# liuhuang31/Megatts2_HierSpeechpp

Hardware: AMD Instinct MI355X
Metric: 16kHz audio samples/sec (whole node) + RTF, HierSpeech++ vocoder batch=32 (higher is better)
Workload: dtype f32; 1 GPU; vocoder-only infer(): 32 utterances x 4 s per GPU (BASELINE.json configs[1]), synthetic weights; batch_per_gpu=32, frames=200, global_batch=32, parallelism=dp1 (contiguous utterance shards of the global batch, one RCCL weight broadcast), launch_mode=hipGraph replay of the captured step

## Files before the change

include/hsp.h:

```cpp
#ifndef HSP_H_
#define HSP_H_

#include <stdint.h>

#ifdef __cplusplus
extern "C" {
#endif
#if defined(__GNUC__) || defined(__clang__)
#pragma GCC visibility push(default)
#endif

#define HSP_VERSION 104
#define HSP_EINVAL (-1)

int hsp_version(void);
const char* hsp_arch(void);


enum {
  HSP_PRO_NONE = 0,
  HSP_PRO_LRELU = 1,
  HSP_PRO_ACT1D = 2,
  HSP_PRO_SILU = 3
};

enum {
  HSP_ACT_NONE = 0,
  HSP_ACT_TANH = 1,
  HSP_ACT_GELU_TANH = 2,
  HSP_ACT_RELU = 3,
  HSP_ACT_MISH = 4,
  HSP_ACT_SILU = 5,
  HSP_ACT_SOFTPLUS = 6,
  HSP_ACT_GELU_ERF = 7
};

enum {
  HSP_ROWS_PLAIN = 0,
  HSP_ROWS_GATE_WN = 1,
  HSP_ROWS_GATE_GLU = 2,
  HSP_ROWS_SHUFFLE = 3
};

enum { HSP_MASK_NONE = 0, HSP_MASK_PRE = 1, HSP_MASK_POST = 2, HSP_MASK_BOTH = 3 };

typedef struct hsp_conv1d_args {
  const float* x;
  int64_t x_bs, x_cs, x_ts;
  int32_t B, Cin, Lin;
  const float* w;
  int32_t K, M, dil, pad, stride;
  const float* zeros;
  int32_t w_ld;
  float* y;
  int64_t y_bs, y_cs;
  int32_t Cout, Lout;
  int32_t ncols;
  int32_t prologue;
  float slope;
  const float* alpha_exp;
  const float* beta_inv;
  const float* filt;
  int32_t rows, gate_half, up, shuf_pad;
  const float* bias;
  const float* cbias;
  int64_t cbias_bs;
  int32_t act;
  const float* mask;
  int64_t mask_bs;
  int32_t mask_mode;
  const float* cscale;
  int64_t cscale_bs;
  float scale;
  const float* res;
  int64_t res_bs, res_cs;
  int32_t accumulate;
  float post_scale;
  int32_t debug;
  const float* ln_c1;
  float ln_eps;
  int32_t split_row;
  int32_t accumulate2;
  int32_t mask_mode2;
  float* y2;
  int64_t y2_bs, y2_cs;
  int64_t res_ts;
  int64_t w_bs;
  int32_t fold_cols;
} hsp_conv1d_args;

int hsp_conv1d_mfma_f32(const hsp_conv1d_args* a, void* stream);
int hsp_conv1d_direct_f32(const hsp_conv1d_args* a, void* stream);
int hsp_conv1d_mfma_plan(const hsp_conv1d_args* a, int32_t out4[4]);

int hsp_act_f32(const float* x, float* y, int64_t n, int32_t act, void* stream);
int hsp_reflect_pad_f32(const float* x, int64_t x_bs, float* y, int32_t B, int32_t L, int32_t pad, void* stream);
int hsp_f0_convert_f32(const float* f0_src, int32_t n_src, const float* f0_trg, int32_t n_trg, float* out, void* stream);

int hsp_reflect_pad_ragged_f32(const float* x, int64_t x_bs, const int64_t* lengths, float* y, int64_t y_bs, int32_t B,
                               int32_t L, int32_t pad, int32_t Lo, void* stream);
int hsp_f0_convert_batch_f32(const float* f0_src, int64_t src_bs, const int64_t* n_src, const float* f0_trg,
                             int64_t trg_bs, const int64_t* n_trg, int32_t nt_max, float* out, int64_t out_bs,
                             int32_t B, int32_t n_max, void* stream);
int hsp_stft_frames_ragged_f32(const float* x, int64_t x_bs, const int64_t* lengths, const float* window, float* frames,
                               int32_t B, int32_t L, int32_t n_fft, int32_t hop, int32_t T, int32_t f_ld, void* stream);
int hsp_abs_max_rows_f32(const float* x, int64_t x_bs, const int64_t* lengths, float* out, int32_t B, int64_t n,
                         void* stream);
int hsp_peak_int16_gains(const float* x, int64_t x_bs, const int64_t* lengths, const float* gains, int16_t* out,
                         int64_t o_bs, int32_t B, int64_t n, void* stream);

int hsp_mag_pha_f32(const float* spec, int64_t s_ld, float* mag, float* pha, int32_t n_freqs, int32_t T, float compress,
                    void* stream);
int hsp_lsigmoid_mul_f32(const float* m, const float* slope, float beta, const float* mag, float* out, int32_t T,
                         int32_t F, void* stream);
int hsp_atan2_f32(const float* y, const float* x, float* out, int64_t n, void* stream);
int hsp_polar_f32(const float* mag, const float* pha, float power, float* re, int64_t re_ld, float* im, int64_t im_ld,
                  int32_t F, int32_t T, void* stream);

int hsp_norm_factor_rows_f32(const float* x, int64_t x_bs, const int64_t* lengths, float* scale, float* inv, int32_t B,
                             int64_t L, void* stream);
int hsp_stft_frames_packed_f32(const float* x, int64_t x_bs, const int64_t* lengths, const float* scale,
                               const float* window, float* frames, const int32_t* seg, const int32_t* seg_host, int32_t B,
                               int64_t L, int32_t n_fft, int32_t hop, int32_t T_tot, int32_t f_ld, void* stream);
int hsp_instnorm_prelu_seg_f32(float* x, int64_t x_cs, int32_t C, int32_t T_tot, int32_t F, const int32_t* seg,
                               const int32_t* seg_host, int32_t B, const float* gamma, const float* beta,
                               const float* slope, float eps, void* stream);
int hsp_zero_gaps_f32(float* x, int64_t x_cs, int32_t C, int32_t T_tot, int32_t F, const int32_t* seg,
                      const int32_t* seg_host, int32_t B, void* stream);
int hsp_dwconv_bn_silu_seg_f32(const float* x, const float* w, const float* bias, const float* bn_weight,
                               const float* bn_bias, const float* bn_mean, const float* bn_var, float bn_eps, float* y,
                               int32_t A, int32_t C, int32_t N, int32_t K, const int32_t* seg, const int32_t* seg_host,
                               int32_t B, void* stream);
int hsp_istft_ola_seg_f32(const float* frames, int64_t f_ld, const float* window, const float* inv, float* out,
                          int64_t out_bs, int64_t n_max, int32_t n_fft, int32_t hop, const int32_t* seg,
                          const int32_t* seg_host, int32_t B, int32_t T_tot, void* stream);

int hsp_act1d_snakebeta_f32(const float* x, float* y, int32_t B, int32_t C, int32_t L,
                            const float* alpha_exp, const float* beta_inv, const float* filt,
                            void* stream);
int hsp_act1d_snakebeta_ragged_f32(const float* x, float* y, int32_t B, int32_t C, int32_t L, const int64_t* lens,
                                   const float* alpha_exp, const float* beta_inv, const float* filt, void* stream);
int hsp_snake_consts_f32(const float* alpha_log, const float* beta_log, float* alpha_exp,
                         float* beta_inv, int32_t C, void* stream);

int hsp_fold_weight_norm_f32(const float* v, const float* g, float* w, int32_t rows, int32_t cols,
                             void* stream);
int hsp_gather_f32(const float* src, const int32_t* map, float* dst, int64_t n, void* stream);

int hsp_sequence_mask_f32(const int64_t* length, float* mask, int32_t B, int32_t T, void* stream);
int hsp_flip_channels_f32(const float* x, float* y, int32_t B, int32_t C, int32_t T, void* stream);
int hsp_sample_prior_f32(const float* stats, const float* noise, const float* mask, float* z,
                         int32_t B, int32_t C, int32_t T, float noise_scale, void* stream);
int hsp_layernorm_mod_f32(const float* x, float* y, int32_t B, int32_t C, int32_t T, float eps,
                          const float* mask, const float* shift, const float* scale, int64_t mod_bs,
                          const float* gamma, const float* beta, void* stream);
typedef struct hsp_mha_args {
  const float *q, *k, *v;
  float* o;
  int64_t q_bs, k_bs, v_bs, o_bs;
  int32_t B, H, D, Tq, Tk;
  float qk_scale;
  const float* mask_q;
  const float* mask_k;
  const float* rel_k;
  const float* rel_v;
  int32_t window;
  int64_t q_cs, k_cs, v_cs, o_cs;
  const float* mask_dense;
  int64_t mask_dense_bs;
} hsp_mha_args;
int hsp_mha_f32(const hsp_mha_args* a, void* stream);
#define HSP_MHA_TOK 0
#define HSP_MHA_MFMA_WHOLE 1
#define HSP_MHA_MFMA_SLAB 2
#define HSP_MHA_MFMA_STREAM 3
#define HSP_MHA_ROW 4
#define HSP_MHA_ROW_STREAM 5
int hsp_mha_plan(const hsp_mha_args* a, int32_t out4[4]);
typedef struct hsp_mha_proj_args {
  const float *q, *k, *v;
  int64_t q_bs, q_cs, k_bs, k_cs, v_bs, v_cs;
  int32_t B, H, D, Tq, Tk;
  float qk_scale;
  const float* wt;
  int32_t M, wt_ld;
  const float* bias;
  const float* mask;
// ... 232 lines not shown
```

megatts2_hierspeechpp_amd/_lib.py:

```python
from __future__ import annotations

import ctypes as C
import os
from typing import Optional

import torch

_HERE = os.path.dirname(os.path.abspath(__file__))
LIB_PATH = os.environ.get("HSP_LIB", os.path.join(_HERE, "libhsp.so"))

PRO_NONE, PRO_LRELU, PRO_ACT1D, PRO_SILU = 0, 1, 2, 3
ACT_NONE, ACT_TANH, ACT_GELU_TANH, ACT_RELU, ACT_MISH, ACT_SILU, ACT_SOFTPLUS, ACT_GELU_ERF = 0, 1, 2, 3, 4, 5, 6, 7
ROWS_PLAIN, ROWS_GATE_WN, ROWS_GATE_GLU, ROWS_SHUFFLE = 0, 1, 2, 3
MASK_NONE, MASK_PRE, MASK_POST, MASK_BOTH = 0, 1, 2, 3
EINVAL = -1
MHA_TOK, MHA_MFMA_WHOLE, MHA_MFMA_SLAB, MHA_MFMA_STREAM, MHA_ROW, MHA_ROW_STREAM = range(6)

_fp = C.c_void_p


class Conv1dArgs(C.Structure):
    _fields_ = [
        ("x", _fp), ("x_bs", C.c_int64), ("x_cs", C.c_int64), ("x_ts", C.c_int64),
        ("B", C.c_int32), ("Cin", C.c_int32), ("Lin", C.c_int32),
        ("w", _fp), ("K", C.c_int32), ("M", C.c_int32), ("dil", C.c_int32), ("pad", C.c_int32), ("stride", C.c_int32),
        ("zeros", _fp), ("w_ld", C.c_int32),
        ("y", _fp), ("y_bs", C.c_int64), ("y_cs", C.c_int64),
        ("Cout", C.c_int32), ("Lout", C.c_int32), ("ncols", C.c_int32),
        ("prologue", C.c_int32), ("slope", C.c_float),
        ("alpha_exp", _fp), ("beta_inv", _fp), ("filt", _fp),
        ("rows", C.c_int32), ("gate_half", C.c_int32), ("up", C.c_int32), ("shuf_pad", C.c_int32),
        ("bias", _fp), ("cbias", _fp), ("cbias_bs", C.c_int64),
        ("act", C.c_int32),
        ("mask", _fp), ("mask_bs", C.c_int64), ("mask_mode", C.c_int32),
        ("cscale", _fp), ("cscale_bs", C.c_int64), ("scale", C.c_float),
        ("res", _fp), ("res_bs", C.c_int64), ("res_cs", C.c_int64),
        ("accumulate", C.c_int32), ("post_scale", C.c_float), ("debug", C.c_int32),
        ("ln_c1", _fp), ("ln_eps", C.c_float),
        ("split_row", C.c_int32), ("accumulate2", C.c_int32), ("mask_mode2", C.c_int32), ("y2", _fp),
        ("y2_bs", C.c_int64), ("y2_cs", C.c_int64), ("res_ts", C.c_int64), ("w_bs", C.c_int64),
        ("fold_cols", C.c_int32),
    ]


class MhaArgs(C.Structure):
    _fields_ = [
        ("q", _fp), ("k", _fp), ("v", _fp), ("o", _fp),
        ("q_bs", C.c_int64), ("k_bs", C.c_int64), ("v_bs", C.c_int64), ("o_bs", C.c_int64),
        ("B", C.c_int32), ("H", C.c_int32), ("D", C.c_int32), ("Tq", C.c_int32), ("Tk", C.c_int32),
        ("qk_scale", C.c_float),
        ("mask_q", _fp), ("mask_k", _fp), ("rel_k", _fp), ("rel_v", _fp), ("window", C.c_int32),
        ("q_cs", C.c_int64), ("k_cs", C.c_int64), ("v_cs", C.c_int64), ("o_cs", C.c_int64),
        ("mask_dense", _fp), ("mask_dense_bs", C.c_int64),
    ]


class MhaProjArgs(C.Structure):
    _fields_ = [
        ("q", _fp), ("k", _fp), ("v", _fp),
        ("q_bs", C.c_int64), ("q_cs", C.c_int64), ("k_bs", C.c_int64), ("k_cs", C.c_int64), ("v_bs", C.c_int64),
        ("v_cs", C.c_int64),
        ("B", C.c_int32), ("H", C.c_int32), ("D", C.c_int32), ("Tq", C.c_int32), ("Tk", C.c_int32),
        ("qk_scale", C.c_float),
        ("wt", _fp), ("M", C.c_int32), ("wt_ld", C.c_int32),
        ("bias", _fp), ("mask", _fp), ("mask_bs", C.c_int64), ("cscale", _fp), ("cscale_bs", C.c_int64),
        ("res", _fp), ("res_bs", C.c_int64), ("res_cs", C.c_int64), ("res_ts", C.c_int64),
        ("y", _fp), ("y_bs", C.c_int64), ("y_cs", C.c_int64), ("y_ts", C.c_int64), ("debug", C.c_int32),
        ("key_len", _fp),
    ]


class DftSegArgs(C.Structure):
    _fields_ = [
        ("x", _fp), ("x_bs", C.c_int64), ("x_cs", C.c_int64),
        ("y", _fp), ("y_bs", C.c_int64), ("y_cs", C.c_int64),
        ("B", C.c_int32), ("C", C.c_int32), ("L", C.c_int32),
        ("k", C.c_int32), ("dil", C.c_int32), ("pad", C.c_int32), ("nseg", C.c_int32), ("Np", C.c_int32),
        ("xf", _fp), ("xf_bs", C.c_int64), ("dft", _fp),
        ("bias", _fp), ("res", _fp), ("res_bs", C.c_int64), ("res_cs", C.c_int64),
        ("accumulate", C.c_int32), ("post_scale", C.c_float),
        ("act_alpha_exp", _fp), ("act_beta_inv", _fp), ("act_filt", _fp), ("prod3", C.c_int32),
        ("act_len", _fp),
    ]


class Cprod3Args(C.Structure):
    _fields_ = [
        ("xf", _fp), ("yf", _fp), ("w", _fp), ("zeros", _fp), ("xf_bs", C.c_int64), ("yf_bs", C.c_int64),
        ("bins", C.c_int32), ("C", C.c_int32), ("Np", C.c_int32), ("debug", C.c_int32),
    ]


class SampleArgs(C.Structure):
    _fields_ = [
        ("temperature", C.c_float), ("top_k", C.c_int32), ("top_p", C.c_float), ("repetition_penalty", C.c_float),
        ("seeds", _fp), ("probs", _fp), ("probs_bs", C.c_int64),
    ]


class PlmDecodeArgs(C.Structure):
    _fields_ = [
        ("x", _fp), ("x_bs", C.c_int64), ("x_cs", C.c_int64),
        ("y", _fp), ("y_bs", C.c_int64), ("y_cs", C.c_int64),
        ("k_cache", _fp), ("v_cache", _fp), ("bs", C.c_int64), ("cs", C.c_int64),
        ("t", C.c_int32), ("B", C.c_int32), ("D", C.c_int32), ("H", C.c_int32), ("F", C.c_int32), ("eps", C.c_float),
        ("g1", _fp), ("b1", _fp), ("wqkv_t", _fp), ("bqkv", _fp), ("wo_t", _fp), ("bo", _fp), ("g2", _fp), ("b2", _fp),
        ("w1_t", _fp), ("c1", _fp), ("w2_t", _fp), ("c2", _fp),
        ("workspace", _fp), ("workspace_bytes", C.c_int64), ("debug", C.c_int32),
    ]


class PlmPrefillAttnArgs(C.Structure):
    _fields_ = [
        ("qkv", _fp), ("q_rs", C.c_int64), ("out", _fp), ("o_rs", C.c_int64),
        ("k_cache", _fp), ("v_cache", _fp), ("cs", C.c_int64),
        ("n", C.c_int32), ("D", C.c_int32), ("H", C.c_int32), ("debug", C.c_int32),
    ]


class ProsodyArgs(C.Structure):
    _fields_ = [
        ("x", _fp), ("x_bs", C.c_int64), ("x_cs", C.c_int64), ("lengths", _fp),
        ("B", C.c_int32), ("D", C.c_int32), ("T", C.c_int32), ("k", C.c_int32), ("w_ld", C.c_int32), ("bins", C.c_int32),
        ("w1a", _fp), ("b1a", _fp), ("w1b", _fp), ("b1b", _fp), ("w2a", _fp), ("b2a", _fp), ("w2b", _fp), ("b2b", _fp),
        ("embed", _fp), ("codes", _fp), ("c_bs", C.c_int64), ("pooled", _fp), ("p_bs", C.c_int64),
    ]


class LimiterArgs(C.Structure):
    _fields_ = [
        ("x", _fp), ("x_bs", C.c_int64), ("lengths", _fp), ("gains", _fp), ("B", C.c_int32), ("n", C.c_int64),
        ("bank", _fp), ("F", C.c_int32), ("Z", C.c_int32), ("W", C.c_int32), ("ceiling", C.c_float),
        ("y", _fp), ("y_bs", C.c_int64), ("min_gain", _fp), ("tp", _fp),
    ]


WSPEC_BLOCK, WSPEC_THREE = 0, 1


SIGNATURES = {
    "hsp_version": (C.c_int, []),
    "hsp_arch": (C.c_char_p, []),
    "hsp_conv1d_mfma_f32": (C.c_int, [C.POINTER(Conv1dArgs), _fp]),
    "hsp_conv1d_direct_f32": (C.c_int, [C.POINTER(Conv1dArgs), _fp]),
    "hsp_conv1d_mfma_plan": (C.c_int, [C.POINTER(Conv1dArgs), C.POINTER(C.c_int32 * 4)]),
    "hsp_act1d_snakebeta_f32": (C.c_int, [_fp, _fp, C.c_int32, C.c_int32, C.c_int32, _fp, _fp, _fp, _fp]),
    "hsp_act1d_snakebeta_ragged_f32": (C.c_int, [_fp, _fp, C.c_int32, C.c_int32, C.c_int32, _fp, _fp, _fp, _fp, _fp]),
    "hsp_snake_consts_f32": (C.c_int, [_fp, _fp, _fp, _fp, C.c_int32, _fp]),
    "hsp_fold_weight_norm_f32": (C.c_int, [_fp, _fp, _fp, C.c_int32, C.c_int32, _fp]),
    "hsp_gather_f32": (C.c_int, [_fp, _fp, _fp, C.c_int64, _fp]),
    "hsp_sequence_mask_f32": (C.c_int, [_fp, _fp, C.c_int32, C.c_int32, _fp]),
    "hsp_flip_channels_f32": (C.c_int, [_fp, _fp, C.c_int32, C.c_int32, C.c_int32, _fp]),
    "hsp_sample_prior_f32": (C.c_int, [_fp, _fp, _fp, _fp, C.c_int32, C.c_int32, C.c_int32, C.c_float, _fp]),
    "hsp_layernorm_mod_f32": (C.c_int, [_fp, _fp, C.c_int32, C.c_int32, C.c_int32, C.c_float, _fp, _fp, _fp,
                                        C.c_int64, _fp, _fp, _fp]),
    "hsp_mha_f32": (C.c_int, [C.POINTER(MhaArgs), _fp]),
    "hsp_mha_plan": (C.c_int, [C.POINTER(MhaArgs), C.POINTER(C.c_int32 * 4)]),
    "hsp_mha_proj_f32": (C.c_int, [C.POINTER(MhaProjArgs), _fp]),
    "hsp_dftseg_fwd_f32": (C.c_int, [C.POINTER(DftSegArgs), _fp]),
    "hsp_dftseg_inv_f32": (C.c_int, [C.POINTER(DftSegArgs), _fp]),
    "hsp_dftseg_tables_f32": (C.c_int, [_fp, _fp]),
    "hsp_dftseg_pair_supported": (C.c_int, [C.POINTER(DftSegArgs), C.POINTER(DftSegArgs)]),
    "hsp_dftseg_pair_f32": (C.c_int, [C.POINTER(DftSegArgs), C.POINTER(DftSegArgs), _fp]),
    "hsp_dftseg_supported": (C.c_int, [C.POINTER(DftSegArgs)]),
    "hsp_cprod3_f32": (C.c_int, [C.POINTER(Cprod3Args), _fp]),
# ... 158 lines not shown
```

megatts2_hierspeechpp_amd/csrc/hsp_conv1d_consume.h:

```cpp
#pragma once

namespace hspconv {

__device__ __forceinline__ unsigned lds_addr(const float* p) {
  return (unsigned)(size_t)(const __attribute__((address_space(3))) float*)p;
}

template <int N, int I = 0>
__device__ __forceinline__ void ds_read_frags(float (&f)[N], unsigned addr) {
  if constexpr (I < N) {
    asm volatile("ds_read_b32 %0, %1 offset:%2" : "=v"(f[I]) : "v"(addr), "n"(I * 128));
    ds_read_frags<N, I + 1>(f, addr);
  }
}

template <int N, int OFF, int I = 0>
__device__ __forceinline__ void ds_read_frags_at(float (&f)[N], unsigned addr) {
  if constexpr (I < N) {
    static_assert(OFF + I * 128 < 65536, "ds_read immediate offsets are 16 bits");
    asm volatile("ds_read_b32 %0, %1 offset:%2" : "=v"(f[I]) : "v"(addr), "n"(OFF + I * 128));
    ds_read_frags_at<N, OFF, I + 1>(f, addr);
  }
}

template <int N, int I = 0>
__device__ __forceinline__ void bind_frags(float (&f)[N]) {
  if constexpr (I < N) {
    asm volatile("" : "+v"(f[I]));
    bind_frags<N, I + 1>(f);
  }
}
template <int NA, int NB>
__device__ __forceinline__ void wait_frags(float (&fa)[NA], float (&fb)[NB]) {
  asm volatile("s_waitcnt lgkmcnt(0)" ::: "memory");
  bind_frags<NA>(fa);
  bind_frags<NB>(fb);
}

template <class C, int EPI, bool ACT, int TM, int TN, bool FOLD = false>
__device__ __forceinline__ void conv_consume(const hsp_conv1d_args& a, const LdsPlan& P, float* const lds, const int b,
                                             const int m0, const int t0, const int p0, const int wm, const int wn,
                                             const int lane, const int nchunks, const int lkc, const int xvec,
                                             const int ks = 0, const int ts0 = 0) {
  static_assert(!FOLD || (TN == 1 && C::kKS == 1 && EPI != HSP_EPI_SHUF && !ACT), "folded columns: one column per lane, plain kernels");
  __builtin_assume(nchunks > 0);
  ConsLane L;
  L.lane = lane, L.l32 = lane & 31, L.half = lane >> 5;
  L.slot = wm * C::kWN + wn;
  L.mw = m0 + wm * (TM * 32), L.wcol = wn * (TN * 32);
  L.b = b, L.t0 = t0, L.ts0 = ts0;
  L.bl = b, L.tw = t0 + L.wcol + L.l32;
  int piece;
  fold_lane<FOLD>(a, b, ts0, L.wcol + L.l32, L.bl, L.tw, piece);
  L.xfold = 8 * piece + 4 - a.pad;

  f32x16 acc[TM][TN];
  {
  const int mw = L.mw, half = L.half, tw = L.tw, bl = L.bl;
  static_assert(C::kKS == 1 || EPI != HSP_EPI_INIT, "a K split with the accumulator-init epilogue would add the residual once per group");
  if constexpr (EPI == HSP_EPI_INIT) {
    const int rcs = (int)a.res_cs, ycs = (int)a.y_cs;
    const int lrow = mw + 4 * half;
    int tcl[TN];
#pragma unroll
    for (int n = 0; n < TN; ++n) tcl[n] = min(tw + n * 32, a.ncols - 1);
    auto init = [&](auto full_tag) __attribute__((always_inline)) {
      constexpr bool FULL = decltype(full_tag)::value;
      auto vec1 = [&](const float* p, int c) __attribute__((always_inline)) -> float {
        if constexpr (FULL) return (p + c)[lrow];
        else return p[min(lrow + c, a.Cout - 1)];
      };
      auto mat = [&](const float* p, int c, int cs, int n) __attribute__((always_inline)) -> float {
        if constexpr (FULL) return (p + c * cs)[lrow * cs + tcl[n]];
        else return p[min(lrow + c, a.Cout - 1) * cs + tcl[n]];
      };
      float add[TM][16];
      if (a.bias) {
        static_for<TM>([&](auto ii) __attribute__((always_inline)) {
          constexpr int i = decltype(ii)::value;
          static_for<16>([&](auto rr) __attribute__((always_inline)) {
            constexpr int r = decltype(rr)::value;
            add[i][r] = vec1(a.bias, i * 32 + HSP_ACC_ROW(r, 0));
          });
        });
      } else {
#pragma unroll
        for (int i = 0; i < TM; ++i)
#pragma unroll
          for (int r = 0; r < 16; ++r) add[i][r] = 0.0f;
      }
      if (a.res) {
        const float* const rb = a.res + (int64_t)bl * a.res_bs;
        static_for<TM>([&](auto ii) __attribute__((always_inline)) {
          constexpr int i = decltype(ii)::value;
          static_for<16>([&](auto rr) __attribute__((always_inline)) {
            constexpr int r = decltype(rr)::value;
            static_for<TN>([&](auto nn) __attribute__((always_inline)) {
              constexpr int n = decltype(nn)::value;
              acc[i][n][r] = mat(rb, i * 32 + HSP_ACC_ROW(r, 0), rcs, n);
            });
          });
        });
      } else {
#pragma unroll
        for (int i = 0; i < TM; ++i)
#pragma unroll
          for (int n = 0; n < TN; ++n)
#pragma unroll
            for (int r = 0; r < 16; ++r) acc[i][n][r] = 0.0f;
      }
      static_for<TM>([&](auto ii) __attribute__((always_inline)) {
        constexpr int i = decltype(ii)::value;
        static_for<TN>([&](auto nn) __attribute__((always_inline)) {
          constexpr int n = decltype(nn)::value;
          static_for<16>([&](auto rr) __attribute__((always_inline)) {
            constexpr int r = decltype(rr)::value;
            acc[i][n][r] += add[i][r];
          });
        });
      });
      if (a.cbias) {
        const float* const cb = a.cbias + (int64_t)bl * a.cbias_bs;
        static_for<TM>([&](auto ii) __attribute__((always_inline)) {
          constexpr int i = decltype(ii)::value;
          static_for<16>([&](auto rr) __attribute__((always_inline)) {
            constexpr int r = decltype(rr)::value;
            const float c = vec1(cb, i * 32 + HSP_ACC_ROW(r, 0));
            static_for<TN>([&](auto nn) __attribute__((always_inline)) {
              constexpr int n = decltype(nn)::value;
              acc[i][n][r] += c;
            });
          });
        });
      }
      if (a.accumulate) {
        const float* const yb = a.y + (int64_t)bl * a.y_bs;
        static_for<TM>([&](auto ii) __attribute__((always_inline)) {
          constexpr int i = decltype(ii)::value;
          static_for<TN>([&](auto nn) __attribute__((always_inline)) {
            constexpr int n = decltype(nn)::value;
            float tmp[16];
            static_for<16>([&](auto rr) __attribute__((always_inline)) {
              constexpr int r = decltype(rr)::value;
              tmp[r] = mat(yb, i * 32 + HSP_ACC_ROW(r, 0), ycs, n);
            });
            __builtin_amdgcn_sched_barrier(0);
            static_for<16>([&](auto rr) __attribute__((always_inline)) {
              constexpr int r = decltype(rr)::value;
              acc[i][n][r] += tmp[r];
            });
            __builtin_amdgcn_sched_barrier(0);
          });
        });
      }
    };
    if (mw + TM * 32 <= a.Cout) {
      init(std::true_type{});
    } else if (mw < a.Cout) {
      init(std::false_type{});
    } else {
#pragma unroll
      for (int i = 0; i < TM; ++i)
#pragma unroll
        for (int n = 0; n < TN; ++n)
#pragma unroll
          for (int r = 0; r < 16; ++r) acc[i][n][r] = 0.0f;
    }
  } else {
#pragma unroll
    for (int i = 0; i < TM; ++i)
#pragma unroll
      for (int j = 0; j < TN; ++j)
#pragma unroll
        for (int r = 0; r < 16; ++r) acc[i][j][r] = 0.0f;
  }
  }
  const int wlane = L.half * C::BM + wm * (TM * 32) + L.l32;
  const int xlane = L.half * P.xwp + L.wcol + L.l32 + (FOLD ? L.xfold : (xvec ? (p0 & 3) : 0));

  {
    constexpr int BM = C::BM;
    const int KC = P.kc;
    const int nsteps = ((a.K * KC) >> 1) / C::kKS;

    HSP_BARRIER(a);
    constexpr int kStepA = 2 * BM * 4;
    constexpr int rowB = 2 * C::XWP * 4;
    const int spanB = (KC >> 1) * rowB;
    const int tapB = 4 * a.dil;
    float fa0[TM], fb0[TN], fa1[TM], fb1[TN];
    auto mma_set = [&](const float (&fa)[TM], const float (&fb)[TN]) __attribute__((always_inline)) {
#pragma unroll
      for (int i = 0; i < TM; ++i)
#pragma unroll
        for (int n = 0; n < TN; ++n)
          acc[i][n] = __builtin_amdgcn_mfma_f32_32x32x2f32(fa[i], fb[n], acc[i][n], 0, 0, 0);
    };
    unsigned aA = lds_addr(lds + wlane);
    unsigned aB = lds_addr(lds + P.xa_off + xlane);
    int offA0 = 0, pairB0 = 0, tapoff0 = 0;
    if constexpr (C::kKS > 1) {
      const int s0 = ks * nsteps;
      offA0 = s0 * kStepA;
      pairB0 = (s0 & ((KC >> 1) - 1)) * rowB;
      tapoff0 = (s0 >> (lkc - 1)) * tapB;
    }
    unsigned va = aA + (unsigned)offA0, vb = aB + (unsigned)(pairB0 + tapoff0);
    const bool run = !HSP_DBG(a, HSP_CV_NO_MFMA);
    if (run) {
      ds_read_frags<TM>(fa0, va);
      ds_read_frags<TN>(fb0, vb);
    }
    for (int c = 0; c < nchunks; ++c) {
      if (!run) {
        HSP_BARRIER(a);
        continue;
      }
      int offA = offA0, pairB = pairB0, tapoff = tapoff0;
      int offB = 0;
      auto advance = [&]() __attribute__((always_inline)) {
        int t;
        asm volatile(
            "s_add_i32 %[oa], %[oa], %[sa]\n\t"
            "s_add_i32 %[pb], %[pb], %[sb]\n\t"
            "s_cmp_eq_u32 %[pb], %[span]\n\t"
            "s_cselect_b32 %[pb], 0, %[pb]\n\t"
            "s_cselect_b32 %[t], %[tap], 0\n\t"
            "s_add_i32 %[to], %[to], %[t]"
            : [oa] "+s"(offA), [pb] "+s"(pairB), [to] "+s"(tapoff), [t] "=&s"(t)
            : [sa] "n"(2 * kStepA), [sb] "n"(2 * rowB), [span] "s"(spanB), [tap] "s"(tapB)
            : "scc");
        offB = pairB + tapoff;
      };
      auto slot_a = [&](bool walk) __attribute__((always_inline)) {
        wait_frags(fa0, fb0);
        __builtin_amdgcn_sched_barrier(0);
        if (walk) advance();
        ds_read_frags_at<TM, kStepA>(fa1, va);
        ds_read_frags_at<TN, rowB>(fb1, vb);
        __builtin_amdgcn_sched_barrier(0);
        mma_set(fa0, fb0);
        __builtin_amdgcn_sched_barrier(0);
      };
      for (int s = 0; s + 2 < nsteps; s += 2) {
        slot_a(true);
        wait_frags(fa1, fb1);
        __builtin_amdgcn_sched_barrier(0);
        va = aA + (unsigned)offA;
        vb = aB + (unsigned)offB;
        ds_read_frags<TM>(fa0, va);
        ds_read_frags<TN>(fb0, vb);
        __builtin_amdgcn_sched_barrier(0);
        mma_set(fa1, fb1);
        __builtin_amdgcn_sched_barrier(0);
      }
      slot_a(false);
      HSP_BARRIER(a);
      bind_frags<TM>(fa1);
      bind_frags<TN>(fb1);
      if (c + 1 < nchunks) {
        const int nb = (c + 1) & 1;
        aA = lds_addr(lds + nb * P.ws_sz + wlane);
        aB = lds_addr(lds + P.xa_off + nb * P.xa_sz + xlane);
        va = aA + (unsigned)offA0;
        vb = aB + (unsigned)(pairB0 + tapoff0);
        __builtin_amdgcn_sched_barrier(0);
        ds_read_frags<TM>(fa0, va);
        ds_read_frags<TN>(fb0, vb);
      }
      __builtin_amdgcn_sched_barrier(0);
      mma_set(fa1, fb1);
      __builtin_amdgcn_sched_barrier(0);
    }
  }

  if constexpr (C::kKS > 1) {
    static_assert(C::kKS == 2, "one partner group per wave");
    float* const red = lds + C::kWM * C::kWN * (32 * 36) + (wm * C::kWN + wn) * (TM * TN * 16 * 64) + lane;
    if (ks > 0) {
      for_acc<TM, TN>([&](auto ii, auto nn, auto rr) __attribute__((always_inline)) {
        constexpr int i = ii, n = nn, r = rr;
        red[((i * TN + n) * 16 + r) * 64] = acc[i][n][r];
      });
    }
    lds_barrier();
    if (ks > 0) return;
    for_acc<TM, TN>([&](auto ii, auto nn, auto rr) __attribute__((always_inline)) {
      constexpr int i = ii, n = nn, r = rr;
      acc[i][n][r] += red[((i * TN + n) * 16 + r) * 64];
    });
  }
  if (HSP_DBG(a, HSP_CV_NO_EPILOGUE)) return;
  if constexpr (EPI == HSP_EPI_INIT) {
    const int mw = L.mw, half = L.half, tw = L.tw, bl = L.bl;
    float* const yb = a.y + (int64_t)bl * a.y_bs;
    const int ycs = (int)a.y_cs;
    const bool full = mw + TM * 32 <= a.Cout &&
                      t0 + wn * (TN * 32) + TN * 32 <= (FOLD ? a.B * a.ncols : a.ncols);
    const float ps = a.post_scale;
    if (full) {
      const int lrow = mw + 4 * half;
      int voff[TN];
#pragma unroll
      for (int n = 0; n < TN; ++n) voff[n] = lrow * ycs + tw + n * 32;
      static_for<TM>([&](auto ii) __attribute__((always_inline)) {
        constexpr int i = decltype(ii)::value;
        static_for<16>([&](auto rr) __attribute__((always_inline)) {
          constexpr int r = decltype(rr)::value;
          float* const yp = yb + (i * 32 + HSP_ACC_ROW(r, 0)) * ycs;
          static_for<TN>([&](auto nn) __attribute__((always_inline)) {
            constexpr int n = decltype(nn)::value;
            if (HSP_DBG(a, HSP_CV_NT_STORES)) __builtin_nontemporal_store(acc[i][n][r] * ps, yp + voff[n]);
            else yp[voff[n]] = acc[i][n][r] * ps;
          });
        });
      });
    } else {
      static_for<TM>([&](auto ii) __attribute__((always_inline)) {
        constexpr int i = decltype(ii)::value;
        static_for<TN>([&](auto nn) __attribute__((always_inline)) {
          constexpr int n = decltype(nn)::value;
          const int t = tw + n * 32;
          static_for<16>([&](auto rr) __attribute__((always_inline)) {
            constexpr int r = decltype(rr)::value;
            const int row = mw + i * 32 + HSP_ACC_ROW(r, half);
            if (row < a.Cout && t < a.ncols) yb[row * ycs + t] = acc[i][n][r] * ps;
          });
        });
      });
    }
  }
  else if constexpr (EPI == HSP_EPI_VEC) epi_vec<FOLD>(a, L, lds, acc);
  else if constexpr (EPI == HSP_EPI_GATE) epi_gate(a, L, acc);
  else if constexpr (EPI == HSP_EPI_SHUF) epi_shuf(a, L, acc);
  else epi_gen(a, L, acc);
}

}
```

megatts2_hierspeechpp_amd/csrc/hsp_conv1d_direct.hip:

```cpp
#include <type_traits>
#include "hsp_device.h"

namespace {

__global__ __launch_bounds__(256) void conv1d_direct_kernel(const hsp_conv1d_args a) {
  const int64_t total = (int64_t)a.B * a.Cout * a.Lout;
  for (int64_t idx = (int64_t)blockIdx.x * blockDim.x + threadIdx.x; idx < total;
       idx += (int64_t)gridDim.x * blockDim.x) {
    const int t = (int)(idx % a.Lout);
    const int64_t r = idx / a.Lout;
    const int co = (int)(r % a.Cout);
    const int b = (int)(r / a.Cout);
    const float* xb = a.x + (int64_t)b * a.x_bs;
    float acc = 0.0f;
    for (int j = 0; j < a.K; ++j) {
      const int p = t * a.stride + j * a.dil - a.pad;
      if (p < 0 || p >= a.Lin) continue;
      const float* wj = a.w + (int64_t)j * a.Cin * a.w_ld + co;
      const float* xp = xb + (int64_t)p * a.x_ts;
      if (a.prologue == HSP_PRO_NONE) {
        float acc4[4] = {0.f, 0.f, 0.f, 0.f};
        int ci = 0;
        for (; ci + 8 <= a.Cin; ci += 8) {
          float wv[8], xv[8];
// ... 33 lines not shown
    f(std::integral_constant<int, N - 1>{});
  }
}

template <int K>
__global__ __launch_bounds__(256) void conv1d_cout1_kernel(const hsp_conv1d_args a, int n_tiles) {
  constexpr int H = (K - 1) / 2, CU = 4;
  __shared__ float ws[C1_MAXW];
  for (int e = threadIdx.x; e < a.Cin * K; e += 256) {
    const int c = e / K, j = e - c * K;
    ws[e] = a.w[((int64_t)j * a.Cin + c) * a.w_ld];
  }
  __syncthreads();
  const int tile = blockIdx.x % n_tiles, b = blockIdx.x / n_tiles;
  const int t = tile * 1024 + 4 * threadIdx.x;
  if (t >= a.Lout) return;
  const int L = a.Lin;
  const float* xb = a.x + (int64_t)b * a.x_bs + t;
  const int64_t xcs = a.x_cs;
  float acc0 = 0.f, acc1 = 0.f, acc2 = 0.f, acc3 = 0.f;
  const bool lo = t - 4 >= 0, hi = t + 4 < L;
  const int offl = lo ? -4 : 0, offh = hi ? 4 : 0;
  const int ngroups = a.Cin / CU;
  for (int g = 0; g < ngroups; ++g) {
    const float* xc = xb + (int64_t)(g * CU) * xcs;
    float4 va[CU], vb[CU], vc[CU];
    c1_static_for<CU>([&](auto uu) __attribute__((always_inline)) {
      constexpr int u = decltype(uu)::value;
      va[u] = *reinterpret_cast<const float4*>(xc + u * xcs + offl);
      vb[u] = *reinterpret_cast<const float4*>(xc + u * xcs);
      vc[u] = *reinterpret_cast<const float4*>(xc + u * xcs + offh);
    });
    c1_static_for<CU>([&](auto uu) __attribute__((always_inline)) {
      constexpr int u = decltype(uu)::value;
      const float w_[12] = {lo ? va[u].x : 0.f, lo ? va[u].y : 0.f, lo ? va[u].z : 0.f, lo ? va[u].w : 0.f,
                            vb[u].x, vb[u].y, vb[u].z, vb[u].w,
                            hi ? vc[u].x : 0.f, hi ? vc[u].y : 0.f, hi ? vc[u].z : 0.f, hi ? vc[u].w : 0.f};
      const float* wc = ws + (g * CU + u) * K;
      c1_static_for<K>([&](auto jj) __attribute__((always_inline)) {
        constexpr int j = decltype(jj)::value;
        const float wj = wc[j];
        acc0 = fmaf(wj, w_[4 + j - H], acc0);
        acc1 = fmaf(wj, w_[5 + j - H], acc1);
        acc2 = fmaf(wj, w_[6 + j - H], acc2);
        acc3 = fmaf(wj, w_[7 + j - H], acc3);
      });
    });
  }
  for (int c = ngroups * CU; c < a.Cin; ++c) {
    const float* xc = xb + (int64_t)c * xcs;
    const float4 va = *reinterpret_cast<const float4*>(xc + offl);
    const float4 vb = *reinterpret_cast<const float4*>(xc);
    const float4 vc = *reinterpret_cast<const float4*>(xc + offh);
    const float w_[12] = {lo ? va.x : 0.f, lo ? va.y : 0.f, lo ? va.z : 0.f, lo ? va.w : 0.f, vb.x, vb.y, vb.z, vb.w,
                          hi ? vc.x : 0.f, hi ? vc.y : 0.f, hi ? vc.z : 0.f, hi ? vc.w : 0.f};
    const float* wc = ws + c * K;
    c1_static_for<K>([&](auto jj) __attribute__((always_inline)) {
      constexpr int j = decltype(jj)::value;
      const float wj = wc[j];
      acc0 = fmaf(wj, w_[4 + j - H], acc0);
      acc1 = fmaf(wj, w_[5 + j - H], acc1);
      acc2 = fmaf(wj, w_[6 + j - H], acc2);
      acc3 = fmaf(wj, w_[7 + j - H], acc3);
    });
  }
  const float bz = a.bias ? a.bias[0] : 0.0f;
  const float sc = a.scale * a.post_scale;
  float4 o;
  o.x = hsp_apply_act(acc0 + bz, a.act) * sc;
  o.y = hsp_apply_act(acc1 + bz, a.act) * sc;
  o.z = hsp_apply_act(acc2 + bz, a.act) * sc;
  o.w = hsp_apply_act(acc3 + bz, a.act) * sc;
  *reinterpret_cast<float4*>(a.y + (int64_t)b * a.y_bs + t) = o;
}

constexpr int LV_WAVES = 8, LV_BB = 8, LV_MAXC = 1024;

__global__ __launch_bounds__(64 * LV_WAVES) void linear_vec_kernel(const hsp_conv1d_args a) {
  __shared__ float xs[LV_BB][LV_MAXC];
  __shared__ float part[LV_WAVES][LV_BB][64];
  const int tid = threadIdx.x, lane = tid & 63, wave = tid >> 6;
  const int co = blockIdx.x * 64 + lane;
  const int b0 = blockIdx.y * LV_BB, nb = min(LV_BB, a.B - b0);
  for (int e = tid; e < nb * a.Cin; e += 64 * LV_WAVES) {
    const int bb = e / a.Cin, ci = e - bb * a.Cin;
    float v = a.x[(int64_t)(b0 + bb) * a.x_bs + (int64_t)ci * a.x_cs];
    if (a.prologue == HSP_PRO_LRELU) v = v > 0.0f ? v : v * a.slope;
    else if (a.prologue == HSP_PRO_SILU) v = v * hsp_sigmoid(v);
    xs[bb][ci] = v;
  }
  __syncthreads();
  const int per = (a.Cin + LV_WAVES - 1) / LV_WAVES;
  const int c0 = wave * per, c1 = min(c0 + per, a.Cin);
  const float* wc = a.w + min(co, a.M - 1);
  float acc[LV_BB];
#pragma unroll
  for (int bb = 0; bb < LV_BB; ++bb) acc[bb] = 0.0f;
  int ci = c0;
  for (; ci + 8 <= c1; ci += 8) {
    float wv[8];
#pragma unroll
    for (int u = 0; u < 8; ++u) wv[u] = wc[(int64_t)(ci + u) * a.w_ld];
#pragma unroll
    for (int u = 0; u < 8; ++u)
#pragma unroll
      for (int bb = 0; bb < LV_BB; ++bb) acc[bb] = fmaf(wv[u], xs[bb][ci + u], acc[bb]);
  }
  for (; ci < c1; ++ci) {
    const float wv = wc[(int64_t)ci * a.w_ld];
#pragma unroll
    for (int bb = 0; bb < LV_BB; ++bb) acc[bb] = fmaf(wv, xs[bb][ci], acc[bb]);
  }
#pragma unroll
  for (int bb = 0; bb < LV_BB; ++bb) part[wave][bb][lane] = acc[bb];
  __syncthreads();
  if (co >= a.Cout) return;
  for (int bb = wave; bb < nb; bb += LV_WAVES) {
    float v = 0.0f;
#pragma unroll
    for (int w = 0; w < LV_WAVES; ++w) v += part[w][bb][lane];
    const int b = b0 + bb;
    if (a.bias) v += a.bias[co];
    if (a.cbias) v += a.cbias[(int64_t)b * a.cbias_bs + co];
    v = hsp_apply_act(v, a.act);
    hsp_epilogue_store(a, b, co, 0, v);
  }
}

bool linear_vec_fast(const hsp_conv1d_args& a) {
  return a.K == 1 && a.Lin == 1 && a.Lout == 1 && a.stride == 1 && a.pad == 0 && a.Cin >= 64 && a.Cin <= LV_MAXC && a.Cout >= 64;
}

bool cout1_fast(const hsp_conv1d_args& a) {
  return a.Cout == 1 && a.stride == 1 && a.dil == 1 && a.K <= 9 && (a.K & 1) && a.pad == (a.K - 1) / 2 && a.x_ts == 1 &&
         a.Lin == a.Lout && (a.Lin & 3) == 0 && (a.x_cs & 3) == 0 && (a.x_bs & 3) == 0 && (a.y_bs & 3) == 0 && hsp_aligned16(a.x) &&
         hsp_aligned16(a.y) && a.prologue == HSP_PRO_NONE && !a.cbias && !a.cscale && !a.res && !a.accumulate &&
         a.mask_mode == HSP_MASK_NONE && (int64_t)a.Cin * a.K <= C1_MAXW;
}

}

extern "C" int hsp_conv1d_direct_f32(const hsp_conv1d_args* ap, void* stream) {
  if (!ap) return HSP_EINVAL;
  const hsp_conv1d_args& a = *ap;
  if (!a.x || !a.w || !a.y) return HSP_EINVAL;
  if (a.B <= 0 || a.Cin <= 0 || a.Lin <= 0 || a.K <= 0 || a.M <= 0 || a.Cout <= 0 || a.Lout <= 0) return HSP_EINVAL;
  if (a.stride < 1 || a.dil < 1 || a.rows != HSP_ROWS_PLAIN || a.Cout > a.M || a.w_ld < a.M) return HSP_EINVAL;
  if (a.prologue != HSP_PRO_NONE && a.prologue != HSP_PRO_LRELU && a.prologue != HSP_PRO_SILU) return HSP_EINVAL;
  if (a.mask_mode != HSP_MASK_NONE && !a.mask) return HSP_EINVAL;
  if (a.res && a.res_ts > 1) return HSP_EINVAL;
  if (a.w_bs) return HSP_EINVAL;
  if (a.ln_c1 || a.split_row) return HSP_EINVAL;
  if (a.fold_cols) return HSP_EINVAL;
  if (linear_vec_fast(a)) {
    const unsigned gx = (unsigned)((a.Cout + 63) / 64), gy = (unsigned)((a.B + LV_BB - 1) / LV_BB);
    if (gy > 65535) return HSP_EINVAL;
    hipLaunchKernelGGL(linear_vec_kernel, dim3(gx, gy), dim3(64 * LV_WAVES), 0, static_cast<hipStream_t>(stream), a);
    return (int)hipGetLastError();
  }
  if (cout1_fast(a)) {
    const int n_tiles = (a.Lout + 1023) / 1024;
    const int64_t nb = (int64_t)n_tiles * a.B;
    if (nb > 0x7fffffff) return HSP_EINVAL;
    const hipStream_t st = static_cast<hipStream_t>(stream);
    switch (a.K) {
      case 1: hipLaunchKernelGGL(conv1d_cout1_kernel<1>, dim3((unsigned)nb), dim3(256), 0, st, a, n_tiles); break;
      case 3: hipLaunchKernelGGL(conv1d_cout1_kernel<3>, dim3((unsigned)nb), dim3(256), 0, st, a, n_tiles); break;
      case 5: hipLaunchKernelGGL(conv1d_cout1_kernel<5>, dim3((unsigned)nb), dim3(256), 0, st, a, n_tiles); break;
      case 7: hipLaunchKernelGGL(conv1d_cout1_kernel<7>, dim3((unsigned)nb), dim3(256), 0, st, a, n_tiles); break;
      default: hipLaunchKernelGGL(conv1d_cout1_kernel<9>, dim3((unsigned)nb), dim3(256), 0, st, a, n_tiles); break;
    }
    return (int)hipGetLastError();
  }
  const int64_t total = (int64_t)a.B * a.Cout * a.Lout;
  int64_t blocks = (total + 255) / 256;
  if (blocks > 262144) blocks = 262144;
  hipLaunchKernelGGL(conv1d_direct_kernel, dim3((unsigned)blocks), dim3(256), 0, static_cast<hipStream_t>(stream), a);
  return (int)hipGetLastError();
}
```

megatts2_hierspeechpp_amd/csrc/hsp_conv1d_epilogue.h:

```cpp
#pragma once

namespace hspconv {

template <int TM, int TN, class F>
__device__ __forceinline__ void for_blocks(F&& f) {
  static_for<TM>([&](auto ii) __attribute__((always_inline)) {
    static_for<TN>([&](auto nn) __attribute__((always_inline)) { f(ii, nn); });
  });
}
template <class F>
__device__ __forceinline__ void for_regs(F&& f) {
  static_for<16>(f);
}
template <int TM, int TN, class F>
__device__ __forceinline__ void for_acc(F&& f) {
  for_blocks<TM, TN>([&](auto ii, auto nn) __attribute__((always_inline)) {
    static_for<16>([&](auto rr) __attribute__((always_inline)) { f(ii, nn, rr); });
  });
}
struct ConsLane {
  int lane, l32, half;
  int slot;
  int mw, wcol;
  int b, t0, ts0;
// ... 92 lines not shown
    constexpr int i = 2 * ih;
    const int mpair = L.mw + i * 32;
    static_for<TN>([&](auto nn) __attribute__((always_inline)) {
      constexpr int n = nn;
      const int t = L.tw + n * 32;
      if (mpair < a.M && t < a.ncols) {
        for_regs([&](auto rr) __attribute__((always_inline)) {
          constexpr int r = rr;
          const int co = (mpair >> 6) * 32 + HSP_ACC_ROW(r, L.half);
          if (co < H) {
            float va = acc[i][n][r], vb = acc[i + 1][n][r];
            if (a.bias) { va += a.bias[co]; vb += a.bias[H + co]; }
            if (a.cbias) {
              va += a.cbias[(int64_t)L.bl * a.cbias_bs + co];
              vb += a.cbias[(int64_t)L.bl * a.cbias_bs + H + co];
            }
            const float v = (a.rows == HSP_ROWS_GATE_WN ? hsp_tanh(va) : va) * hsp_sigmoid(vb);
            hsp_epilogue_store(a, L.bl, co, t, v);
          }
        });
      }
    });
  });
}

__device__ __forceinline__ void convtr_row(const hsp_conv1d_args& a, float up_inv, int m, int& co, int& phase) {
  co = (int)(((float)m + 0.5f) * up_inv);
  phase = m - co * a.up;
}

template <int TM, int TN>
__device__ __forceinline__ void epi_shuf_vec(const hsp_conv1d_args& a, const ConsLane& L, const f32x16 (&acc)[TM][TN]) {
  typedef float st4 __attribute__((ext_vector_type(4), aligned(4)));
  typedef float st2 __attribute__((ext_vector_type(2), aligned(4)));
  const float sc = a.scale * a.post_scale;
  const int upl = a.up == 4 ? 2 : 1;
  static_for<TM>([&](auto ii) __attribute__((always_inline)) {
    constexpr int i = ii;
    float* yrow[4][2];
    float bz[4][2];
    bool rok[4][2];
#pragma unroll
    for (int q = 0; q < 4; ++q)
#pragma unroll
      for (int c2 = 0; c2 < 2; ++c2) {
        const int m = L.mw + i * 32 + 8 * q + 4 * L.half + 2 * c2;
        const int co = m >> upl;
        rok[q][c2] = m < a.M && co < a.Cout;
        yrow[q][c2] = a.y + (int64_t)L.bl * a.y_bs + (int64_t)(rok[q][c2] ? co : 0) * a.y_cs;
        bz[q][c2] = (rok[q][c2] && a.bias) ? a.bias[co] : 0.0f;
      }
    static_for<TN>([&](auto nn) __attribute__((always_inline)) {
      constexpr int n = nn;
      const int t = L.tw + n * 32;
      if (t < a.ncols) {
        const int to0 = a.up * t - a.shuf_pad;
        const bool inside = to0 >= 0 && to0 + a.up <= a.Lout;
        static_for<4>([&](auto qq) __attribute__((always_inline)) {
          constexpr int q = qq;
          if (a.up == 4) {
            if (rok[q][0]) {
              const st4 v = {(acc[i][n][4 * q] + bz[q][0]) * sc, (acc[i][n][4 * q + 1] + bz[q][0]) * sc,
                             (acc[i][n][4 * q + 2] + bz[q][0]) * sc, (acc[i][n][4 * q + 3] + bz[q][0]) * sc};
              if (inside) *reinterpret_cast<st4*>(yrow[q][0] + to0) = v;
              else {
#pragma unroll
                for (int ph = 0; ph < 4; ++ph)
                  if (to0 + ph >= 0 && to0 + ph < a.Lout) yrow[q][0][to0 + ph] = v[ph];
              }
            }
          } else {
#pragma unroll
            for (int c2 = 0; c2 < 2; ++c2) {
              if (rok[q][c2]) {
                const st2 v = {(acc[i][n][4 * q + 2 * c2] + bz[q][c2]) * sc, (acc[i][n][4 * q + 2 * c2 + 1] + bz[q][c2]) * sc};
                if (inside) *reinterpret_cast<st2*>(yrow[q][c2] + to0) = v;
                else {
#pragma unroll
                  for (int ph = 0; ph < 2; ++ph)
                    if (to0 + ph >= 0 && to0 + ph < a.Lout) yrow[q][c2][to0 + ph] = v[ph];
                }
              }
            }
          }
        });
      }
    });
  });
}

template <int TM, int TN>
__device__ __forceinline__ void epi_shuf(const hsp_conv1d_args& a, const ConsLane& L, const f32x16 (&acc)[TM][TN]) {
  if ((a.up == 4 || a.up == 2) && !HSP_DBG(a, HSP_CV_SHUF_SCALAR)) return epi_shuf_vec(a, L, acc);
  const float up_inv = 1.0f / (float)a.up;
  static_for<TM>([&](auto ii) __attribute__((always_inline)) {
    constexpr int i = ii;
    float* yrow[16];
    float bz[16];
    int toff[16];
#pragma unroll
    for (int r = 0; r < 16; ++r) {
      const int m = L.mw + i * 32 + HSP_ACC_ROW(r, L.half);
      int co, phase;
      convtr_row(a, up_inv, m, co, phase);
      const bool ok = m < a.M && co < a.Cout;
      toff[r] = ok ? phase - a.shuf_pad : -(1 << 30);
      yrow[r] = a.y + (int64_t)L.bl * a.y_bs + (int64_t)(ok ? co : 0) * a.y_cs;
      bz[r] = (ok && a.bias) ? a.bias[co] : 0.0f;
    }
    static_for<TN>([&](auto nn) __attribute__((always_inline)) {
      constexpr int n = nn;
      const int t = L.tw + n * 32;
      if (t < a.ncols) {
        for_regs([&](auto rr) __attribute__((always_inline)) {
          constexpr int r = rr;
          const int to = a.up * t + toff[r];
          if (to >= 0 && to < a.Lout) yrow[r][to] = (acc[i][n][r] + bz[r]) * a.scale * a.post_scale;
        });
      }
    });
  });
}

template <int TM, int TN>
__device__ __forceinline__ void epi_gen(const hsp_conv1d_args& a, const ConsLane& L, const f32x16 (&acc)[TM][TN]) {
  const float up_inv = a.rows == HSP_ROWS_SHUFFLE ? 1.0f / (float)a.up : 1.0f;
  for_blocks<TM, TN>([&](auto ii, auto nn) __attribute__((always_inline)) {
    constexpr int i = ii, n = nn;
    const int t = L.tw + n * 32;
    if (t < a.ncols) {
      for_regs([&](auto rr) __attribute__((always_inline)) {
        constexpr int r = rr;
        const int m = L.mw + i * 32 + HSP_ACC_ROW(r, L.half);
        int co = m, to = t;
        bool ok = m < a.M;
        if (a.rows == HSP_ROWS_SHUFFLE) {
          co = (int)(((float)m + 0.5f) * up_inv);
          to = a.up * t + (m - co * a.up) - a.shuf_pad;
          ok = ok && to >= 0 && to < a.Lout;
        }
        ok = ok && co < a.Cout;
        if (ok) {
          float v = acc[i][n][r];
          if (a.bias) v += a.bias[co];
          if (a.cbias) v += a.cbias[(int64_t)L.bl * a.cbias_bs + co];
          v = hsp_apply_act(v, a.act);
          hsp_epilogue_store(a, L.bl, co, to, v);
        }
      });
    }
  });
}

}
```

megatts2_hierspeechpp_amd/csrc/hsp_conv1d_mfma.hip:

```cpp
#include "hsp_conv1d_mfma_kernel.h"
#include "hsp_token_gemm.h"

namespace {
using namespace hspconv;

int validate(const hsp_conv1d_args& a) {
  if (!a.x || !a.w || !a.y) return HSP_EINVAL;
#ifndef HSP_TUNING
  if (a.debug != 0) return HSP_EINVAL;
#endif
  if (a.B <= 0 || a.Cin <= 0 || a.Lin <= 0 || a.K <= 0 || a.M <= 0 || a.Cout <= 0 || a.Lout <= 0 || a.ncols <= 0)
    return HSP_EINVAL;
  if (a.stride != 1 || (a.M & 3) || (a.w_ld & 3) || a.w_ld < a.M || a.dil < 1) return HSP_EINVAL;
  if ((reinterpret_cast<uintptr_t>(a.w) & 15) != 0 || a.w_bs < 0 || (a.w_bs & 3)) return HSP_EINVAL;
  if (a.w_bs && (a.ln_c1 || a.split_row || (a.res && a.res_ts > 1))) return HSP_EINVAL;
  if ((int64_t)a.K * a.Cin * a.w_ld >= (1ll << 31)) return HSP_EINVAL;
  if ((int64_t)a.Cin * a.x_cs + (int64_t)a.Lin * a.x_ts >= (1ll << 31) || a.x_cs < 0 || a.x_ts < 0) return HSP_EINVAL;
  if (a.y_cs < 0 || (int64_t)a.Cout * a.y_cs + a.Lout >= (1ll << 31)) return HSP_EINVAL;
  if (a.res && (a.res_cs < 0 || (int64_t)a.Cout * a.res_cs + a.Lout >= (1ll << 31))) return HSP_EINVAL;
  if (a.res_ts < 0 || (a.res && a.res_ts > 1 && (int64_t)a.Cout * a.res_cs + (int64_t)a.Lout * a.res_ts >= (1ll << 31))) return HSP_EINVAL;
  if (a.prologue == HSP_PRO_ACT1D && (!a.alpha_exp || !a.beta_inv || !a.filt || a.x_ts != 1)) return HSP_EINVAL;
  if (!a.zeros || (reinterpret_cast<uintptr_t>(a.zeros) & 15) != 0) return HSP_EINVAL;
  if (a.prologue != HSP_PRO_NONE && a.prologue != HSP_PRO_LRELU && a.prologue != HSP_PRO_ACT1D) return HSP_EINVAL;
  if (a.mask_mode != HSP_MASK_NONE && !a.mask) return HSP_EINVAL;
  if (a.fold_cols != 0 && a.fold_cols != 1) return HSP_EINVAL;
  if (a.rows == HSP_ROWS_GATE_WN || a.rows == HSP_ROWS_GATE_GLU) {
    if (a.gate_half <= 0 || (a.gate_half & 31) || a.M != 2 * a.gate_half || a.Cout != a.gate_half) return HSP_EINVAL;
    if (a.prologue == HSP_PRO_ACT1D) return HSP_EINVAL;
  } else if (a.rows == HSP_ROWS_SHUFFLE) {
    if (a.up <= 0 || a.up > 16 || a.M < a.Cout * a.up || a.M - a.Cout * a.up > 3 || a.M > (1 << 16)) return HSP_EINVAL;
  } else if (a.rows != HSP_ROWS_PLAIN) {
    return HSP_EINVAL;
  }
  return 0;
}

int dispatch(const hsp_conv1d_args& a, hipStream_t s, int32_t* plan_out) {
  const bool gated = a.rows == HSP_ROWS_GATE_WN || a.rows == HSP_ROWS_GATE_GLU;
  const bool act = a.prologue == HSP_PRO_ACT1D;
  const bool short_seq = hsp_tile_count(a, 128, 128) <= 128;
  if (a.res && a.res_ts > 1) {
    if (a.fold_cols) return HSP_EINVAL;
    const int e = hsp_rgemm_try(a, s, plan_out);
    return e >= 0 ? e : HSP_EINVAL;
  }
  if (a.K == 1 && !a.w_bs && !HSP_TG_DBG(a, HSP_TG_OFF)) {
    const int e = hsp_bgemm_try(a, s, plan_out);
    if (e >= 0) return e;
  }
  hsp_conv1d_args plain = a;
  plain.fold_cols = 0;
  int32_t probe[4];
  if ((short_seq || a.ln_c1 || a.split_row || HSP_TG_DBG(a, HSP_TG_RG_ANY_SIZE)) && !a.w_bs && !HSP_TG_DBG(a, HSP_TG_OFF)) {
    if (a.fold_cols && hsp_rgemm_try(plain, nullptr, probe) >= 0) return HSP_EINVAL;
    const int e = hsp_rgemm_try(a, s, plan_out);
    if (e >= 0) return e;
  }
  if (a.ln_c1 || a.split_row) return HSP_EINVAL;
  int epi = select_epilogue(a);
  if (act && epi != HSP_EPI_INIT) epi = HSP_EPI_GEN;
  if ((a.K - 1) * a.dil + 3 > 64)
    return gated ? hsp_conv_tile_S64GW(a, epi, act, s, plan_out) : hsp_conv_tile_S64W(a, epi, act, s, plan_out);
#ifdef HSP_TUNING
  if (!gated && HSP_DBG(a, HSP_CV_TILE_M128)) return hsp_conv_tile_M128(a, epi, act, s, plan_out);
  if (!gated && HSP_DBG(a, HSP_CV_TILE_M64)) return hsp_conv_tile_M64(a, epi, act, s, plan_out);
  if (!gated && HSP_DBG(a, HSP_CV_TILE_S64)) return hsp_conv_tile_S64(a, epi, act, s, plan_out);
  if (!gated && HSP_DBG(a, HSP_CV_TILE_M64P)) return hsp_conv_tile_M64P(a, epi, act, s, plan_out);
#endif
  if (short_seq) {
    if (gated) {
      const int64_t t128 = hsp_tile_count(a, 64, 128);
      if ((t128 <= 48 || (HSP_DBG(a, HSP_CV_S64G2_512) && t128 <= 512)) && !HSP_DBG(a, HSP_CV_NO_S64G2)) {
        if (a.fold_cols && hsp_conv_tile_S64G2(plain, epi, act, nullptr, probe) != HSP_EINVAL) return HSP_EINVAL;
        const int e = hsp_conv_tile_S64G2(a, epi, act, s, plan_out);
        if (e != HSP_EINVAL) return e;
      }
      return hsp_conv_tile_S64G(a, epi, act, s, plan_out);
    }
    if (a.M > 32) return hsp_conv_tile_S64(a, epi, act, s, plan_out);
    return hsp_conv_tile_S32(a, epi, act, s, plan_out);
  }
  if (gated) return hsp_conv_tile_M128(a, epi, act, s, plan_out);
  if (a.M > 64) return hsp_conv_tile_M128(a, epi, act, s, plan_out);
  if (a.M > 32) return act ? hsp_conv_tile_M64(a, epi, act, s, plan_out) : hsp_conv_tile_M64P(a, epi, act, s, plan_out);
  return act ? hsp_conv_tile_M32(a, epi, act, s, plan_out) : hsp_conv_tile_M32P(a, epi, act, s, plan_out);
}

}

extern "C" int hsp_conv1d_mfma_f32(const hsp_conv1d_args* a, void* stream) {
  if (!a) return HSP_EINVAL;
  if (int e = validate(*a)) return e;
  return dispatch(*a, static_cast<hipStream_t>(stream), nullptr);
}

extern "C" int hsp_conv1d_mfma_plan(const hsp_conv1d_args* a, int32_t out4[4]) {
  if (!a || !out4) return HSP_EINVAL;
  if (int e = validate(*a)) return e;
  return dispatch(*a, nullptr, out4);
}
```

megatts2_hierspeechpp_amd/csrc/hsp_conv1d_mfma_kernel.h:

```cpp
#pragma once
#include <atomic>
#include <type_traits>
#include "hsp_device.h"

typedef float f32x16 __attribute__((ext_vector_type(16)));

#ifdef HSP_TUNING
#define HSP_DBG(a, bit) (((a).debug & (bit)) != 0)
#else
#define HSP_DBG(a, bit) false
#endif
enum : int32_t {
  HSP_CV_ONE_CHUNK = 1,
  HSP_CV_NO_MFMA = 2,
  HSP_CV_NO_EPILOGUE = 16,
  HSP_CV_NO_INIT = 32,
  HSP_CV_NO_XVEC = 64,
  HSP_CV_TILE_M128 = 256,
  HSP_CV_NO_FAST_STAGE = 512,
  HSP_CV_TILE_M64 = 1024,
  HSP_CV_NO_BARRIER = 2048,
  HSP_CV_TILE_S64 = 4096,
  HSP_CV_TILE_M64P = 8192,
  HSP_CV_XCD_GROUPS = 16384,
  HSP_CV_NO_TAIL = 32768,
  HSP_CV_NT_STORES = 65536,
  HSP_CV_SHUF_SCALAR = 262144,
  HSP_CV_NO_HALF_CU = 1 << 21,
  HSP_CV_HALF_CU_ANY = 1 << 26,
  HSP_CV_NO_S64G2 = 1 << 27,
  HSP_CV_S64G2_512 = 1 << 28,
  HSP_CV_DEEP_K3 = 1 << 29,
};

enum {
  HSP_EPI_INIT = 0,
  HSP_EPI_VEC = 1,
  HSP_EPI_GATE = 2,
  HSP_EPI_SHUF = 3,
  HSP_EPI_GEN = 4
};

namespace hspconv {

template <int WM, int WN, int TM, int TN, int NPW_, int MINW_, int XSLACK_ = 64, int KS_ = 1, bool FOLD_ = false>
struct Cfg {
  static constexpr bool kFOLD = FOLD_;
  static constexpr int kKS = KS_;
  static constexpr int NCW = WM * WN * KS_;
  static constexpr int kWM = WM, kWN = WN, kTM = TM, kTN = TN;
  static constexpr int BM = WM * TM * 32;
  static constexpr int BN = WN * TN * 32;
  static constexpr int NPW = NPW_;
  static constexpr int NPT = NPW_ * 64;
  static constexpr int THREADS = 64 * (WM * WN * KS_ + NPW_);
  static constexpr int MINW = MINW_;
  static constexpr int XWP = BN + XSLACK_;
};

struct LdsPlan {
  int kc, lkc;
  int rpw;
  int xw;
  int xwp;
  int xrw;
  int xrwp;
  int a2w;
  int ws_sz, xa_sz, scr_sz;
  int xa_off, scr_off, total;
};

template <class C>
__host__ __device__ inline LdsPlan make_plan(int K, int dil, int prologue, int lkc) {
  LdsPlan p;
  p.lkc = lkc;
  p.kc = 1 << lkc;
  p.rpw = (p.kc + C::NPW - 1) / C::NPW;
  p.xw = C::BN + (K - 1) * dil;
  p.xwp = C::XWP;
  p.xrw = p.xw + 10;
  p.xrwp = (p.xrw + 63) & ~63;
  p.a2w = 2 * p.xw + 10;
  p.ws_sz = K * p.kc * C::BM;
  p.xa_sz = p.kc * p.xwp;
  p.scr_sz = prologue == HSP_PRO_ACT1D ? 2 * p.rpw * p.xrwp + ((p.a2w + 3) & ~3) : 0;
  p.xa_off = 2 * p.ws_sz;
  p.scr_off = p.xa_off + 2 * p.xa_sz;
  p.total = p.scr_off + C::NPW * p.scr_sz;
  return p;
}

template <int N, class F>
__device__ __forceinline__ void static_for(F&& f) {
  if constexpr (N > 0) {
    static_for<N - 1>(f);
    f(std::integral_constant<int, N - 1>{});
  }
}

__device__ __forceinline__ void lds_barrier() {
  asm volatile("s_waitcnt lgkmcnt(0)" ::: "memory");
  __builtin_amdgcn_s_barrier();
  asm volatile("" ::: "memory");
}
#define HSP_BARRIER(a) do { if (!HSP_DBG(a, HSP_CV_NO_BARRIER)) lds_barrier(); } while (0)

__device__ __forceinline__ void wave_lds_fence() { asm volatile("s_waitcnt lgkmcnt(0)" ::: "memory"); }

__device__ __forceinline__ void fold_col(int col, int ts0, int T, int& i, int& t) {
  i = 0;
  t = ts0 + col;
  while (t >= T) {
    t -= T;
    ++i;
  }
}

}

#include "hsp_conv1d_produce.h"
#include "hsp_conv1d_epilogue.h"
#include "hsp_conv1d_consume.h"

namespace hspconv {


template <class C, int EPI, bool ACT>
constexpr bool has_tail_path() {
  return EPI == HSP_EPI_INIT && !ACT && C::kWM * C::kWN == 4 && C::kTM * C::kWM == 4 && C::kTN * C::kWN == 4;
}

template <class C, int EPI, bool ACT, bool FOLD = false>
__global__ __launch_bounds__(C::THREADS, C::MINW) void conv1d_mfma_kernel(const hsp_conv1d_args a, const int n_mt,
                                                                          const int n_nt, const int lkc,
                                                                          const int xvec, const int sched) {
  extern __shared__ __attribute__((aligned(16))) float lds[];
  constexpr int BM = C::BM, BN = C::BN, TM = C::kTM, TN = C::kTN;
  const LdsPlan P = make_plan<C>(a.K, a.dil, ACT ? HSP_PRO_ACT1D : HSP_PRO_NONE, lkc);
  const int KC = P.kc;

  int mt, ct;
  {
    const int g = sched & 255;
    const int bid = blockIdx.x;
    if (g == 0) {
      mt = bid % n_mt;
      ct = bid / n_mt;
    } else {
      const int x = bid & 7, q = bid >> 3;
      const int groups_m = n_mt / g, nx = 8 / groups_m;
      mt = (x % groups_m) * g + q % g;
      ct = (q / g) * nx + x / groups_m;
      if (ct >= n_nt * a.B) return;
    }
  }
  int nt, b;
  bool tail_tile = false;
  if constexpr (FOLD) {
    nt = ct;
    b = (nt * BN) / a.ncols;
  } else if (sched >> 8) {
    const int n_main = (n_nt - 1) * a.B;
    if (ct < n_main) {
      nt = ct % (n_nt - 1);
      b = ct / (n_nt - 1);
    } else {
      nt = n_nt - 1;
      b = ct - n_main;
      tail_tile = true;
    }
  } else {
    nt = ct % n_nt;
    b = ct / n_nt;
  }
  const int m0 = mt * BM, t0 = nt * BN;
  const int p0 = t0 - a.pad;
  const int ts0 = FOLD ? t0 - b * a.ncols : 0;

  const int wave = __builtin_amdgcn_readfirstlane(threadIdx.x >> 6);
  const int lane = threadIdx.x & 63;
  const int nchunks = (a.Cin + KC - 1) >> lkc;

  if (wave >= C::NCW) {
    const int pw = wave - C::NCW;
    using PR = Prod<C>;
    const float* const wb = a.w + (int64_t)b * a.w_bs;
    const ProdArgs pa{wb, a.zeros, a.alpha_exp, a.beta_inv, a.filt, a.K, a.Cin, a.Lin, a.M, a.w_ld, (int)a.x_cs,
                      (int)a.x_ts, a.prologue, a.slope};
    const float* xb = a.x + (int64_t)b * a.x_bs;
    float* const Ws0 = lds;
    float* const Xa0 = lds + P.xa_off;
    if constexpr (FOLD) {
      const int T = a.ncols;
      const int ngrp = (BN + 8 * ((BN + T - 1) / T + 1)) >> 2;
      int q = 4 * lane + ts0, piece = 0;
      while (q >= T + 8) {
        q -= T + 8;
        ++piece;
      }
      const bool inside = b + piece < a.B && q >= 4 && q < T + 4;
      const float* const xl = inside ? a.x + (int64_t)(b + piece) * a.x_bs + (q - 4) : a.zeros;
      const int xs = inside ? (int)a.x_cs : 0;
      const bool wfast = m0 + BM <= a.M && (a.Cin & (KC - 1)) == 0;
      const float* const wtile = wb + m0;
      const unsigned wofs = PR::w_lane_ofs(lane, a.w_ld);
      auto stage = [&](int c0, float* Ws, float* Xa) __attribute__((always_inline)) {
        if (wfast) PR::dma_w_fast(wtile, a.w_ld, a.Cin, a.K, P, Ws, c0, pw, wofs);
        else PR::dma_w(pa, P, Ws, c0, m0, pw, lane);
        PR::dma_x_fold(xl, xs, a.zeros, a.Cin, P, Xa, c0, pw, lane < ngrp);
        wait_vm0();
        if (a.prologue == HSP_PRO_LRELU) PR::lrelu_x(pa, P, Xa, pw, lane);
      };
      stage(0, Ws0, Xa0);
      HSP_BARRIER(a);
      for (int c = 0; c < nchunks; ++c) {
        const int nb = (c + 1) & 1;
        if (c + 1 < nchunks && !HSP_DBG(a, HSP_CV_ONE_CHUNK)) stage((c + 1) << lkc, Ws0 + nb * P.ws_sz, Xa0 + nb * P.xa_sz);
        HSP_BARRIER(a);
      }
    } else if constexpr (!ACT) {
      const int p0a = p0 & ~3;
      const bool fast = xvec && m0 + BM <= a.M && (a.Cin & (KC - 1)) == 0 && !HSP_DBG(a, HSP_CV_NO_FAST_STAGE);
      if (fast) {
        const float* const wtile = wb + m0;
        const float* const xtile = xb + p0a;
        const int xcs = (int)a.x_cs;
        const unsigned wofs = PR::w_lane_ofs(lane, a.w_ld);
        if (p0a < 0 || p0a + 4 * ((P.xw + 3 + 3) >> 2) > a.Lin) PR::zero_x_rows(P, Xa0, pw, lane);
        PR::dma_w_fast(wtile, a.w_ld, a.Cin, a.K, P, Ws0, 0, pw, wofs);
        PR::dma_x16_fast(xtile, xcs, a.Lin, P, Xa0, 0, p0a, pw, lane);
        wait_vm0();
        if (a.prologue == HSP_PRO_LRELU) PR::lrelu_x(pa, P, Xa0, pw, lane);
        HSP_BARRIER(a);
        for (int c = 0; c < nchunks; ++c) {
          const int nb = (c + 1) & 1;
          if (c + 1 < nchunks && !HSP_DBG(a, HSP_CV_ONE_CHUNK)) {
            PR::dma_w_fast(wtile, a.w_ld, a.Cin, a.K, P, Ws0 + nb * P.ws_sz, (c + 1) << lkc, pw, wofs);
            PR::dma_x16_fast(xtile, xcs, a.Lin, P, Xa0 + nb * P.xa_sz, (c + 1) << lkc, p0a, pw, lane);
            wait_vm0();
            if (a.prologue == HSP_PRO_LRELU) PR::lrelu_x(pa, P, Xa0 + nb * P.xa_sz, pw, lane);
          }
          HSP_BARRIER(a);
        }
        return;
      }
      PR::dma_w(pa, P, Ws0, 0, m0, pw, lane);
      if (xvec) PR::dma_x16(pa, P, Xa0, xb, 0, p0a, pw, lane); else PR::dma_x(pa, P, Xa0, xb, 0, p0, pw, lane);
      wait_vm0();
      if (a.prologue == HSP_PRO_LRELU) PR::lrelu_x(pa, P, Xa0, pw, lane);
      HSP_BARRIER(a);
      for (int c = 0; c < nchunks; ++c) {
        const int nb = (c + 1) & 1;
        if (c + 1 < nchunks && !HSP_DBG(a, HSP_CV_ONE_CHUNK)) {
          PR::dma_w(pa, P, Ws0 + nb * P.ws_sz, (c + 1) << lkc, m0, pw, lane);
          if (xvec) PR::dma_x16(pa, P, Xa0 + nb * P.xa_sz, xb, (c + 1) << lkc, p0a, pw, lane);
          else PR::dma_x(pa, P, Xa0 + nb * P.xa_sz, xb, (c + 1) << lkc, p0, pw, lane);
          wait_vm0();
          if (a.prologue == HSP_PRO_LRELU) PR::lrelu_x(pa, P, Xa0 + nb * P.xa_sz, pw, lane);
        }
        HSP_BARRIER(a);
      }
    } else {
      float* const scr = lds + P.scr_off + pw * P.scr_sz;
      float* const a2 = scr + 2 * P.rpw * P.xrwp;
      const int rsz = P.rpw * P.xrwp;
      PR::dma_raw(pa, P, scr, xb, 0, p0, pw, lane);
      PR::dma_w(pa, P, Ws0, 0, m0, pw, lane);
      wait_vm0();
      PR::act_rows(pa, P, scr, a2, Xa0, 0, p0, pw, lane);
      if (nchunks > 1) PR::dma_raw(pa, P, scr + rsz, xb, KC, p0, pw, lane);
      wait_vm0();
      HSP_BARRIER(a);
      for (int c = 0; c < nchunks; ++c) {
        const int nb = (c + 1) & 1;
        if (c + 1 < nchunks && !HSP_DBG(a, HSP_CV_ONE_CHUNK)) {
          PR::dma_w(pa, P, Ws0 + nb * P.ws_sz, (c + 1) << lkc, m0, pw, lane);
          if (c + 2 < nchunks) PR::dma_raw(pa, P, scr + (c & 1) * rsz, xb, (c + 2) << lkc, p0, pw, lane);
          PR::act_rows(pa, P, scr + nb * rsz, a2, Xa0 + nb * P.xa_sz, (c + 1) << lkc, p0, pw, lane);
          wait_vm0();
        }
        HSP_BARRIER(a);
      }
    }
    return;
  }

  if constexpr (has_tail_path<C, EPI, ACT>()) {
    if (tail_tile) {
      conv_consume<C, EPI, ACT, 1, 1>(a, P, lds, b, m0, t0, p0, wave, 0, lane, nchunks, lkc, xvec);
      return;
    }
  }
  if constexpr (FOLD) {
    conv_consume<C, EPI, ACT, TM, TN, true>(a, P, lds, b, m0, t0, p0, wave / C::kWN, wave % C::kWN, lane, nchunks, lkc, xvec, 0, ts0);
  } else if constexpr (C::kKS > 1) {
    const int ks = wave / (C::kWM * C::kWN), w2 = wave % (C::kWM * C::kWN);
    conv_consume<C, EPI, ACT, TM, TN>(a, P, lds, b, m0, t0, p0, w2 / C::kWN, w2 % C::kWN, lane, nchunks, lkc, xvec, ks);
  } else {
    conv_consume<C, EPI, ACT, TM, TN>(a, P, lds, b, m0, t0, p0, wave / C::kWN, wave % C::kWN, lane, nchunks, lkc, xvec);
  }
}

constexpr int kMaxLdsBytes = 160 * 1024;
constexpr int kLdsTarget = 80 * 1024;

template <class C>
int pick_lkc(const hsp_conv1d_args& a, int lds_limit) {
  const bool act = a.prologue == HSP_PRO_ACT1D;
  if (C::BN + (a.K - 1) * a.dil + 3 > C::XWP) return -1;
  int cin_p2 = 2;
  while ((1 << cin_p2) < a.Cin && cin_p2 < 6) ++cin_p2;
  for (int lkc = cin_p2; lkc >= 2; --lkc) {
    const LdsPlan P = make_plan<C>(a.K, a.dil, a.prologue, lkc);
    if (P.total * (int)sizeof(float) > lds_limit) continue;
    if (P.kc < Prod<C>::RPI) continue;
    if (C::kKS > 1 && (((a.K * P.kc) >> 1) % (2 * C::kKS) != 0 || P.total < C::kWM * C::kWN * (32 * 36 + C::kTM * C::kTN * 16 * 64))) continue;
    if (act && P.rpw > 2) continue;
    return lkc;
  }
  return -1;
}

template <class C, int EPI, bool ACT>
constexpr bool has_fold_path() {
  return C::kFOLD && !ACT && EPI != HSP_EPI_SHUF;
}

inline bool window_dma16(const hsp_conv1d_args& a, bool act) {
  return !act && a.x_ts == 1 && (a.Lin & 3) == 0 && (a.x_cs & 3) == 0 && (a.x_bs & 3) == 0 && hsp_aligned16(a.x) &&
         !HSP_DBG(a, HSP_CV_NO_XVEC);
}

template <class C>
bool fold_fits(const hsp_conv1d_args& a, bool xvec) {
  const int T = a.ncols;
  if (!a.fold_cols || a.B < 2 || !xvec || (T & 3) || (T % C::BN) == 0 || a.w_bs) return false;
  if (a.Lin != T || a.Lout != T || a.pad > 4 || (a.K - 1) * a.dil - a.pad > 4) return false;
  if (C::BN + 8 * ((C::BN + T - 1) / T + 1) > C::XWP) return false;
  return (int64_t)a.B * T <= 0x3fffffff;
}

template <class C, int EPI, bool ACT>
int launch_one(const hsp_conv1d_args& a, hipStream_t s, int32_t* plan_out) {
  if (a.fold_cols && !has_fold_path<C, EPI, ACT>()) return HSP_EINVAL;
  const int64_t tiles = (int64_t)((a.M + C::BM - 1) / C::BM) * ((a.ncols + C::BN - 1) / C::BN) * a.B;
  const bool deep_k3 = HSP_DBG(a, HSP_CV_DEEP_K3) && a.K <= 3;
  const bool two_per_cu = !deep_k3 && (C::MINW * 256 >= 2 * C::THREADS || ((tiles > 256 || HSP_DBG(a, HSP_CV_HALF_CU_ANY)) && tiles <= 512 && !HSP_DBG(a, HSP_CV_NO_HALF_CU)));
  int lkc = pick_lkc<C>(a, two_per_cu ? kLdsTarget : kMaxLdsBytes);
  if (lkc < 0) lkc = pick_lkc<C>(a, kMaxLdsBytes);
  if (lkc < 0) return HSP_EINVAL;
  int lds_bytes = make_plan<C>(a.K, a.dil, a.prologue, lkc).total * (int)sizeof(float);
  if (plan_out) {
    plan_out[0] = C::BM; plan_out[1] = C::BN; plan_out[2] = 1 << lkc; plan_out[3] = lds_bytes;
    return 0;
  }
  const int n_mt = (a.M + C::BM - 1) / C::BM;
  const int n_nt = (a.ncols + C::BN - 1) / C::BN;
  const int64_t n_ct = (int64_t)n_nt * a.B;
  int g = 0;
  if (HSP_DBG(a, HSP_CV_XCD_GROUPS) && n_mt >= 1 && n_mt <= 8 && (8 % n_mt) == 0) {
    const int64_t slab = (int64_t)a.K * a.Cin * C::BM * (int64_t)sizeof(float);
    g = 1;
    for (int cand = n_mt; cand > 1; cand >>= 1)
      if (n_mt % cand == 0 && (int64_t)cand * slab <= (int64_t)3200 * 1024) { g = cand; break; }
  }
  const int rem = a.ncols - (n_nt - 1) * C::BN;
  const int tail = (has_tail_path<C, EPI, ACT>() && n_nt >= 2 && rem <= 32 && !HSP_DBG(a, HSP_CV_NO_TAIL)) ? 1 : 0;
  int64_t blocks = (int64_t)n_mt * n_ct;
  if (g > 0) {
    const int nx = 8 / (n_mt / g);
    blocks = 8 * (int64_t)g * ((n_ct + nx - 1) / nx);
  }
  if (blocks <= 0 || blocks > 0x7fffffff) return HSP_EINVAL;
  const int sched = g | (tail << 8);
  auto kern = conv1d_mfma_kernel<C, EPI, ACT>;
  static hsp_lds_flags flags;
  if (lds_bytes > 32 * 1024)
    if (int e = hsp_raise_lds_limit(reinterpret_cast<const void*>(kern), kMaxLdsBytes, flags)) return e;
  if (EPI == HSP_EPI_VEC && lds_bytes < C::NCW * 32 * 36 * 4) lds_bytes = C::NCW * 32 * 36 * 4;
  const bool xvec = window_dma16(a, ACT);
  if constexpr (has_fold_path<C, EPI, ACT>()) {
    if (fold_fits<C>(a, xvec)) {
      auto kfold = conv1d_mfma_kernel<C, EPI, ACT, true>;
      static hsp_lds_flags fflags;
      if (lds_bytes > 32 * 1024)
        if (int e = hsp_raise_lds_limit(reinterpret_cast<const void*>(kfold), kMaxLdsBytes, fflags)) return e;
      const int n_vt = (int)(((int64_t)a.B * a.ncols + C::BN - 1) / C::BN);
      hipLaunchKernelGGL(kfold, dim3((unsigned)(n_mt * n_vt)), dim3(C::THREADS), lds_bytes, s, a, n_mt, n_vt, lkc, 1, 0);
      return (int)hipGetLastError();
    }
  }
  hipLaunchKernelGGL(kern, dim3((unsigned)blocks), dim3(C::THREADS), lds_bytes, s, a, n_mt, n_nt, lkc, xvec ? 1 : 0, sched);
  return (int)hipGetLastError();
}

inline int select_epilogue(const hsp_conv1d_args& a) {
  if (a.rows == HSP_ROWS_GATE_WN || a.rows == HSP_ROWS_GATE_GLU) return HSP_EPI_GATE;
  const bool pointwise = a.act != HSP_ACT_NONE || a.mask_mode != HSP_MASK_NONE || a.cscale;
  if (a.rows == HSP_ROWS_SHUFFLE)
    return (!pointwise && !a.cbias && !a.res && !a.accumulate) ? HSP_EPI_SHUF : HSP_EPI_GEN;
  if (!pointwise && a.scale == 1.0f && !HSP_DBG(a, HSP_CV_NO_INIT)) return HSP_EPI_INIT;
  const bool vec = (a.ncols & 3) == 0 && hsp_aligned16(a.y) && (a.y_bs & 3) == 0 && (a.y_cs & 3) == 0 &&
                   (!a.res || (hsp_aligned16(a.res) && (a.res_bs & 3) == 0 && (a.res_cs & 3) == 0)) &&
                   (a.mask_mode == HSP_MASK_NONE || (hsp_aligned16(a.mask) && (a.mask_bs & 3) == 0));
  return vec ? HSP_EPI_VEC : HSP_EPI_GEN;
}

using M128 = Cfg<2, 2, 2, 2, 4, 4>;
using M64 = Cfg<1, 4, 2, 2, 8, 3>;
using M32 = Cfg<1, 4, 1, 4, 8, 3>;
using M64P = Cfg<1, 4, 2, 2, 4, 4>;
using M32P = Cfg<1, 4, 1, 4, 4, 4>;
using S64 = Cfg<2, 2, 1, 1, 4, 2, 64, 1, true>;
using S64G = Cfg<1, 4, 2, 1, 4, 2, 64, 1, true>;
using S32 = Cfg<1, 4, 1, 1, 4, 2>;
using S64W = Cfg<2, 2, 1, 1, 4, 2, 128>;
using S64GW = Cfg<1, 4, 2, 1, 4, 2, 128>;
using S64G2 = Cfg<1, 2, 2, 1, 4, 2, 64, 2>;

}

#define HSP_TILE_LIST(X) X(M128) X(M64) X(M32) X(M64P) X(M32P) X(S64) X(S64G) X(S32) X(S64W) X(S64GW) X(S64G2)
#define HSP_TILE_DECL(name) \
  int hsp_conv_tile_##name(const hsp_conv1d_args& a, int epi, bool act, hipStream_t s, int32_t* plan_out);
HSP_TILE_LIST(HSP_TILE_DECL)
#undef HSP_TILE_DECL
```

megatts2_hierspeechpp_amd/csrc/hsp_conv1d_tile.hip:

```cpp
#include "hsp_conv1d_mfma_kernel.h"

#ifndef HSP_TILE
#error "compile with -DHSP_TILE=<M128|M64|M32|M64P|M32P|S64|S64G|S32|S64W|S64GW|S64G2>"
#endif

namespace {
using namespace hspconv;
using T = HSP_TILE;

template <class A, class B>
constexpr bool same = std::is_same<A, B>::value;

template <int EPI, bool ACT>
constexpr bool supported() {
  if (same<T, S64G> || same<T, S64GW> || same<T, S64G2>) return EPI == HSP_EPI_GATE && !ACT;
  if (same<T, M64> || same<T, M32>) return ACT && (EPI == HSP_EPI_INIT || EPI == HSP_EPI_GEN);
  if (ACT) return (same<T, M128> || same<T, S64> || same<T, S64W> || same<T, S32>) && (EPI == HSP_EPI_INIT || EPI == HSP_EPI_GEN);
  if (EPI == HSP_EPI_GATE) return same<T, M128>;
  if (EPI == HSP_EPI_SHUF) return true;
  return true;
}

template <int EPI, bool ACT>
int try_one(const hsp_conv1d_args& a, hipStream_t s, int32_t* plan_out) {
  if constexpr (supported<EPI, ACT>()) return launch_one<T, EPI, ACT>(a, s, plan_out);
  else return HSP_EINVAL;
}

template <int EPI>
int by_act(const hsp_conv1d_args& a, bool act, hipStream_t s, int32_t* plan_out) {
  return act ? try_one<EPI, true>(a, s, plan_out) : try_one<EPI, false>(a, s, plan_out);
}
}

#define HSP_CAT_(a, b) a##b
#define HSP_CAT(a, b) HSP_CAT_(a, b)

int HSP_CAT(hsp_conv_tile_, HSP_TILE)(const hsp_conv1d_args& a, int epi, bool act, hipStream_t s, int32_t* plan_out) {
  switch (epi) {
    case HSP_EPI_INIT: return by_act<HSP_EPI_INIT>(a, act, s, plan_out);
    case HSP_EPI_VEC: return by_act<HSP_EPI_VEC>(a, act, s, plan_out);
    case HSP_EPI_GATE: return by_act<HSP_EPI_GATE>(a, act, s, plan_out);
    case HSP_EPI_SHUF: return by_act<HSP_EPI_SHUF>(a, act, s, plan_out);
    case HSP_EPI_GEN: return by_act<HSP_EPI_GEN>(a, act, s, plan_out);
    default: return HSP_EINVAL;
  }
}
```

megatts2_hierspeechpp_amd/csrc/hsp_pointwise.hip:

```cpp
#include "hsp_rows.h"

namespace {

inline unsigned loop_grid(int64_t n) { return hsp_flat_grid(n, 256, 1048576); }

constexpr int ACT_TILE = 1024;
constexpr int ACT_THREADS = 256;
constexpr int ACT_HALO = 8;

typedef float act_f32x2 __attribute__((ext_vector_type(2)));

__global__ __launch_bounds__(ACT_THREADS) void act1d_kernel(const float* __restrict__ x, float* __restrict__ y, int C,
                                                            int L, const float* __restrict__ alpha_exp,
                                                            const float* __restrict__ beta_inv,
                                                            const float* __restrict__ filt, int n_tiles) {
  __shared__ __attribute__((aligned(16))) float raw[ACT_TILE + 2 * ACT_HALO];
  __shared__ __attribute__((aligned(16))) float a2[2 * ACT_TILE + 16];
  const int tile = blockIdx.x % n_tiles;
  const int row = blockIdx.x / n_tiles;
  const int c = row % C;
  const int p0 = tile * ACT_TILE;
  const float* xrow = x + (int64_t)row * L;
  float* yrow = y + (int64_t)row * L;
  const float kf = alpha_exp[c] * 0.318309886183790672f, kb = 0.5f * beta_inv[c];
  const int n_out = min(ACT_TILE, L - p0);
  const int tid = threadIdx.x;
  const bool vec = ((L & 3) == 0) && ((reinterpret_cast<uintptr_t>(x) & 15) == 0) &&
                   ((reinterpret_cast<uintptr_t>(y) & 15) == 0);
  const int nraw = n_out + 2 * ACT_HALO;
  if (vec && p0 >= ACT_HALO && p0 + n_out + ACT_HALO <= L) {
    for (int v = tid; v < nraw / 4; v += ACT_THREADS)
      *reinterpret_cast<float4*>(raw + 4 * v) = *reinterpret_cast<const float4*>(xrow + p0 - ACT_HALO + 4 * v);
  } else {
    for (int s = tid; s < nraw; s += ACT_THREADS) raw[s] = xrow[hsp_clampi(p0 - ACT_HALO + s, 0, L - 1)];
  }
  __syncthreads();
  const int a2w = 2 * n_out + 10;
  const int mlo = 2 * p0 - 5;
  if (mlo >= 0 && mlo + a2w <= 2 * L) {
    const int npair = (a2w - 1) >> 1;
    float hu[12];
#pragma unroll
    for (int t = 0; t < 12; ++t) hu[t] = filt[t];
    for (int i = 2 * tid; i < npair; i += 2 * ACT_THREADS) {
      float xv[8];
#pragma unroll
      for (int t = 0; t < 8; ++t) xv[t] = raw[i + 3 + t];
      act_f32x2 u0 = {0.0f, 0.0f}, u1 = {0.0f, 0.0f};
#pragma unroll
      for (int t = 0; t < 6; ++t) {
        const act_f32x2 hh = {hu[11 - 2 * t], hu[10 - 2 * t]};
        const act_f32x2 x0 = {xv[t], xv[t + 1]};
        const act_f32x2 x1 = {xv[t + 1], xv[t + 2]};
        u0 = __builtin_elementwise_fma(x0, hh, u0);
        u1 = __builtin_elementwise_fma(x1, hh, u1);
      }
      u0 = u0 * 2.0f;
      u1 = u1 * 2.0f;
      a2[2 * i + 1] = hsp_snake_hw(u0.x, kf, kb);
      a2[2 * i + 2] = hsp_snake_hw(u0.y, kf, kb);
      if (i + 1 < npair) {
        a2[2 * i + 3] = hsp_snake_hw(u1.x, kf, kb);
        a2[2 * i + 4] = hsp_snake_hw(u1.y, kf, kb);
      }
    }
    if (tid < 2) {
      const float* xr_ = tid ? raw + n_out + 7 : raw + 3;
      float uu = 0.0f;
#pragma unroll
      for (int t = 0; t < 6; ++t) uu = fmaf(xr_[t], tid ? filt[11 - 2 * t] : filt[10 - 2 * t], uu);
      a2[tid ? a2w - 1 : 0] = hsp_snake_hw(2.0f * uu, kf, kb);
    }
  } else {
    for (int s = tid; s < a2w; s += ACT_THREADS) {
      const int m = hsp_clampi(mlo + s, 0, 2 * L - 1);
      const int q = m >> 1, odd = m & 1;
      const float* xr_ = raw + (q - 3 + odd) - (p0 - ACT_HALO);
      float u = 0.0f;
#pragma unroll
      for (int t = 0; t < 6; ++t) u = fmaf(xr_[t], odd ? filt[10 - 2 * t] : filt[11 - 2 * t], u);
      a2[s] = hsp_snake_hw(2.0f * u, kf, kb);
    }
  }
  __syncthreads();
  float hd[12];
#pragma unroll
  for (int t = 0; t < 12; ++t) hd[t] = filt[12 + t];
  if (vec && (n_out & 3) == 0) {
    for (int v = tid; v < n_out / 4; v += ACT_THREADS) {
      const act_f32x2* ar = reinterpret_cast<const act_f32x2*>(a2 + 8 * v);
      act_f32x2 w[9];
#pragma unroll
      for (int k = 0; k < 9; ++k) w[k] = ar[k];
      float o[4];
#pragma unroll
      for (int q = 0; q < 4; ++q) {
        act_f32x2 acc = {0.0f, 0.0f};
#pragma unroll
        for (int k = 0; k < 6; ++k) {
          const act_f32x2 hh = {hd[2 * k], hd[2 * k + 1]};
          acc = __builtin_elementwise_fma(w[q + k], hh, acc);
        }
        o[q] = acc.x + acc.y;
      }
      *reinterpret_cast<float4*>(yrow + p0 + 4 * v) = make_float4(o[0], o[1], o[2], o[3]);
    }
  } else {
    for (int s = tid; s < n_out; s += ACT_THREADS) {
      const act_f32x2* ar = reinterpret_cast<const act_f32x2*>(a2 + 2 * s);
      act_f32x2 acc = {0.0f, 0.0f};
#pragma unroll
      for (int k = 0; k < 6; ++k) {
        const act_f32x2 hh = {hd[2 * k], hd[2 * k + 1]};
        acc = __builtin_elementwise_fma(ar[k], hh, acc);
      }
      yrow[p0 + s] = acc.x + acc.y;
    }
  }
}

constexpr int ACT2_SEG = 496;
constexpr int ACT2_WAVES = 4;
constexpr int ACT2_ITEMS = 4;
constexpr int ACT2_RAW = 512;
constexpr int ACT2_A2 = 1040;

__device__ __forceinline__ void act2_compiler_fence() { asm volatile("" ::: "memory"); }

struct Act2Item {
  int p0, n_out, c;
  int64_t row_off;
};

__device__ __forceinline__ Act2Item act2_item(unsigned w, int nseg, int C, int L) {
  const unsigned row = w / (unsigned)nseg;
  const int seg = (int)(w - row * (unsigned)nseg);
  Act2Item it;
  it.p0 = seg * ACT2_SEG;
  it.n_out = min(ACT2_SEG, L - it.p0);
  it.c = (int)(row % (unsigned)C);
  it.row_off = (int64_t)row * L;
  return it;
}

__device__ __forceinline__ void act2_load(const float* __restrict__ x, const Act2Item& it, int L, int lane,
                                          float4 (&rv)[2]) {
  const float* xrow = x + it.row_off;
#pragma unroll
  for (int k = 0; k < 2; ++k) {
    const int idx = it.p0 - 8 + 4 * (lane + 64 * k);
    rv[k] = *reinterpret_cast<const float4*>(xrow + hsp_clampi(idx, 0, L - 4));
  }
}

__device__ __forceinline__ int act2_row_len(const int64_t* __restrict__ lens, unsigned w, int nseg, int C, int L) {
  const unsigned b = (w / (unsigned)nseg) / (unsigned)C;
  return (int)hsp_clamp_len(lens[b], L, 1);
}

template <bool RAG>
__global__ __launch_bounds__(64 * ACT2_WAVES) void act1d_seg_kernel(const float* __restrict__ x, float* __restrict__ y,
                                                                    int C, int L, const float* __restrict__ alpha_exp,
                                                                    const float* __restrict__ beta_inv,
                                                                    const float* __restrict__ filt, int nseg,
                                                                    unsigned nwork, const int64_t* __restrict__ lens) {
  __shared__ __attribute__((aligned(16))) float raw_all[ACT2_WAVES][ACT2_RAW];
  __shared__ __attribute__((aligned(16))) float a2_all[ACT2_WAVES][ACT2_A2];
  const int wave = __builtin_amdgcn_readfirstlane(threadIdx.x >> 6);
  const int lane = threadIdx.x & 63;
  const unsigned w0 = (blockIdx.x * ACT2_WAVES + wave) * ACT2_ITEMS;
  if (w0 >= nwork) return;
  const unsigned w1 = min(w0 + ACT2_ITEMS, nwork);
  float* raw = raw_all[wave];
  float* a2 = a2_all[wave];
  act_f32x2 hu[6], hd[6];
#pragma unroll
  for (int i = 0; i < 6; ++i) {
    hu[i] = act_f32x2{2.0f * filt[10 - 2 * i], 2.0f * filt[11 - 2 * i]};
    hd[i] = act_f32x2{filt[12 + 2 * i], filt[13 + 2 * i]};
  }

  Act2Item cur = act2_item(w0, nseg, C, L);
  float4 rv[2];
  act2_load(x, cur, L, lane, rv);
  int lb = L;
  float rl = 0.0f;
  if constexpr (RAG) {
    lb = act2_row_len(lens, w0, nseg, C, L);
    rl = x[cur.row_off + lb - 1];
  }
  constexpr int NC = (ACT2_SEG / 2 + 63) / 64;
  float2 yo[NC];
  float* yprev = nullptr;
  int nprev = 0;
  auto flush = [&]() __attribute__((always_inline)) {
#pragma unroll
    for (int it = 0; it < NC; ++it) {
      const int l2 = lane + 64 * it;
      if (2 * l2 < nprev) __builtin_nontemporal_store(act_f32x2{yo[it].x, yo[it].y}, reinterpret_cast<act_f32x2*>(yprev + 2 * l2));
    }
  };
  for (unsigned w = w0; w < w1; ++w) {
    const int p0 = cur.p0, n_out = cur.n_out;
    const int lbc = lb;
    const float rlc = rl;
    const int n_in = RAG ? max(0, min(n_out, lbc - p0)) : n_out;
    float* yrow = y + cur.row_off;
    const float kf = alpha_exp[cur.c] * 0.318309886183790672f, kb = 0.5f * beta_inv[cur.c];
#pragma unroll
    for (int k = 0; k < 2; ++k) {
      const int v = lane + 64 * k;
      const int idx = p0 - 8 + 4 * v;
      float4 t = rv[k];
      t = idx < 0 ? make_float4(t.x, t.x, t.x, t.x) : t;
      t = idx >= L ? make_float4(t.w, t.w, t.w, t.w) : t;
      if constexpr (RAG) {
        t.x = idx >= lbc ? rlc : t.x;
        t.y = idx + 1 >= lbc ? rlc : t.y;
        t.z = idx + 2 >= lbc ? rlc : t.z;
        t.w = idx + 3 >= lbc ? rlc : t.w;
      }
      *reinterpret_cast<float4*>(raw + 4 * v) = t;
    }
    act2_compiler_fence();
    if (yprev) flush();
    if (w + 1 < w1) {
      cur = act2_item(w + 1, nseg, C, L);
      act2_load(x, cur, L, lane, rv);
      if constexpr (RAG) {
        lb = act2_row_len(lens, w + 1, nseg, C, L);
        rl = x[cur.row_off + lb - 1];
      }
    }
    act2_compiler_fence();

    const int npairs = (2 * n_out + 13) >> 2;
#pragma unroll 2
    for (int pi = lane; pi < npairs; pi += 64) {
      const act_f32x2* rp = reinterpret_cast<const act_f32x2*>(raw + 2 * pi + 2);
      const act_f32x2 r0 = rp[0], r1 = rp[1], r2 = rp[2], r3 = rp[3];
      const float xv[7] = {r0.y, r1.x, r1.y, r2.x, r2.y, r3.x, r3.y};
      act_f32x2 u0 = {0.0f, 0.0f}, u1 = {0.0f, 0.0f};
#pragma unroll
      for (int i = 0; i < 6; ++i) {
        u0 = __builtin_elementwise_fma(act_f32x2{xv[i], xv[i]}, hu[i], u0);
        u1 = __builtin_elementwise_fma(act_f32x2{xv[i + 1], xv[i + 1]}, hu[i], u1);
      }
      *reinterpret_cast<float4*>(a2 + 4 * pi) = make_float4(hsp_snake_hw(u0.x, kf, kb), hsp_snake_hw(u0.y, kf, kb),
                                                            hsp_snake_hw(u1.x, kf, kb), hsp_snake_hw(u1.y, kf, kb));
    }
    act2_compiler_fence();
    if constexpr (RAG) {
      const int e = 2 * (lbc - p0) + 4;
      const bool tail = e >= 0 && e < 2 * n_out + 9;
      if (p0 == 0 || tail) {
        if (p0 == 0 && lane < 5) a2[lane] = a2[5];
        if (tail && lane >= 8 && lane < 13) a2[e + lane - 7] = a2[e];
        act2_compiler_fence();
      }
    } else if (p0 == 0 || p0 + n_out == L) {
      if (p0 == 0 && lane < 5) a2[lane] = a2[5];
      if (p0 + n_out == L && lane >= 8 && lane < 13) a2[2 * n_out + lane - 3] = a2[2 * n_out + 4];
      act2_compiler_fence();
    }

#pragma unroll
    for (int it = 0; it < NC; ++it) {
      const int l2 = lane + 64 * it;
      if (2 * l2 >= n_out) continue;
      const float4* ap = reinterpret_cast<const float4*>(a2 + 4 * l2);
      const float4 q0 = ap[0], q1 = ap[1], q2 = ap[2];
      const act_f32x2 q3 = *reinterpret_cast<const act_f32x2*>(a2 + 4 * l2 + 12);
      const act_f32x2 aw[7] = {{q0.x, q0.y}, {q0.z, q0.w}, {q1.x, q1.y}, {q1.z, q1.w}, {q2.x, q2.y}, {q2.z, q2.w}, q3};
      act_f32x2 s0 = {0.0f, 0.0f}, s1 = {0.0f, 0.0f};
#pragma unroll
      for (int k = 0; k < 6; ++k) {
        s0 = __builtin_elementwise_fma(aw[k], hd[k], s0);
        s1 = __builtin_elementwise_fma(aw[k + 1], hd[k], s1);
      }
      yo[it] = make_float2(s0.x + s0.y, s1.x + s1.y);
      if constexpr (RAG) {
        yo[it].x = 2 * l2 < n_in ? yo[it].x : 0.0f;
        yo[it].y = 2 * l2 + 1 < n_in ? yo[it].y : 0.0f;
      }
    }
    yprev = yrow + p0;
    nprev = n_out;
    act2_compiler_fence();
  }
  flush();
}

__global__ void snake_consts_kernel(const float* al, const float* bl, float* ea, float* binv, int C) {
  const int i = blockIdx.x * blockDim.x + threadIdx.x;
  if (i < C) {
    ea[i] = expf(al[i]);
    binv[i] = 1.0f / (expf(bl[i]) + 1e-9f);
  }
}

__global__ __launch_bounds__(256) void fold_weight_norm_kernel(const float* __restrict__ v, const float* __restrict__ g,
                                                               float* __restrict__ w, int rows, int cols) {
  const int row = blockIdx.x * 4 + (threadIdx.x >> 6);
  const int lane = threadIdx.x & 63;
  if (row >= rows) return;
  const float* vr = v + (int64_t)row * cols;
  float ss = 0.0f;
  for (int i = lane; i < cols; i += 64) ss = fmaf(vr[i], vr[i], ss);
#pragma unroll
  for (int o = 32; o > 0; o >>= 1) ss += __shfl_xor(ss, o, 64);
  const float sc = g[row] / sqrtf(ss);
  float* wr = w + (int64_t)row * cols;
  for (int i = lane; i < cols; i += 64) wr[i] = vr[i] * sc;
}

__global__ void gather_kernel(const float* __restrict__ src, const int32_t* __restrict__ map, float* __restrict__ dst,
                              int64_t n) {
  for (int64_t i = (int64_t)blockIdx.x * blockDim.x + threadIdx.x; i < n; i += (int64_t)gridDim.x * blockDim.x) {
    const int32_t m = map[i];
    dst[i] = m >= 0 ? src[m] : 0.0f;
  }
}

__global__ void sequence_mask_kernel(const int64_t* length, float* mask, int B, int T) {
  const int i = blockIdx.x * blockDim.x + threadIdx.x;
  if (i < B * T) mask[i] = (i % T) < length[i / T] ? 1.0f : 0.0f;
}

__global__ void flip_channels_kernel(const float* __restrict__ x, float* __restrict__ y, int B, int C, int T) {
  const int64_t n = (int64_t)B * C * T;
  for (int64_t i = (int64_t)blockIdx.x * blockDim.x + threadIdx.x; i < n; i += (int64_t)gridDim.x * blockDim.x) {
    const int t = (int)(i % T);
    const int64_t r = i / T;
    const int c = (int)(r % C);
    const int64_t b = r / C;
    y[i] = x[(b * C + (C - 1 - c)) * T + t];
  }
}

__global__ void sample_prior_kernel(const float* __restrict__ stats, const float* __restrict__ noise,
                                    const float* __restrict__ mask, float* __restrict__ z, int B, int C, int T,
                                    float noise_scale) {
  const int64_t n = (int64_t)B * C * T;
  for (int64_t i = (int64_t)blockIdx.x * blockDim.x + threadIdx.x; i < n; i += (int64_t)gridDim.x * blockDim.x) {
    const int t = (int)(i % T);
    const int64_t r = i / T;
    const int c = (int)(r % C);
    const int64_t b = r / C;
    const float m = stats[(b * 2 * C + c) * T + t];
    const float logs = stats[(b * 2 * C + C + c) * T + t];
    z[i] = (m + noise[i] * expf(logs) * noise_scale) * mask[b * T + t];
  }
}

__global__ void mask_mul_kernel(const float* __restrict__ x, const float* __restrict__ mask, float* __restrict__ y,
                                int B, int C, int T) {
  const int64_t n = (int64_t)B * C * T;
  for (int64_t i = (int64_t)blockIdx.x * blockDim.x + threadIdx.x; i < n; i += (int64_t)gridDim.x * blockDim.x) {
    const int t = (int)(i % T);
    const int64_t b = i / ((int64_t)C * T);
    y[i] = x[i] * mask[b * T + t];
  }
}

template <bool RAG>
__global__ void linear_interp_kernel(const float* __restrict__ x, float* __restrict__ y, int64_t rows, int C, int Lin,
                                     int Lout, float scale, const int64_t* __restrict__ lin,
                                     const int64_t* __restrict__ lout) {
  const int64_t n = rows * Lout;
  for (int64_t i = (int64_t)blockIdx.x * blockDim.x + threadIdx.x; i < n; i += (int64_t)gridDim.x * blockDim.x) {
    const int t = (int)(i % Lout);
    const int64_t r = i / Lout;
    int lb_in = Lin;
    if constexpr (RAG) {
      lb_in = (int)hsp_row_len(lin, r / C, Lin, 1);
      if (t >= (int)hsp_row_len(lout, r / C, Lout)) {
        y[i] = 0.0f;
        continue;
      }
    }
    float src = fmaf(scale, (float)t + 0.5f, -0.5f);
    src = src < 0.0f ? 0.0f : src;
    const int i0 = RAG ? min((int)src, lb_in - 1) : (int)src;
    const int i1 = i0 + (i0 < lb_in - 1 ? 1 : 0);
    const float l1 = src - (float)i0, l0 = 1.0f - l1;
    const float* xr = x + r * Lin;
    y[i] = l0 * xr[i0] + l1 * xr[i1];
  }
}

__global__ void act_kernel(const float* x, float* y, int64_t n, int act) {
  for (int64_t i = (int64_t)blockIdx.x * blockDim.x + threadIdx.x; i < n; i += (int64_t)gridDim.x * blockDim.x)
    y[i] = hsp_apply_act(x[i], act);
}

__global__ __launch_bounds__(256) void reflect_pad_kernel(const float* __restrict__ x, int64_t x_bs,
                                                          const int64_t* __restrict__ lengths, float* __restrict__ y,
                                                          int64_t y_bs, int B, int L, int pad, int Lo) {
  const int t = blockIdx.x * 256 + threadIdx.x;
  if (t >= Lo) return;
  for (int b = blockIdx.y; b < B; b += gridDim.y) {
    const int n = (int)hsp_row_len(lengths, b, L);
    float v = 0.0f;
    if (n > 0 && t < n + 2 * pad) v = x[(int64_t)b * x_bs + hsp_reflect(t - pad, n)];
    y[(int64_t)b * y_bs + t] = v;
  }
}

__global__ __launch_bounds__(256) void f0_convert_kernel(const float* src, int ns, const float* trg, int nt, float* out) {
  hsp_f0_convert_row(src, ns, trg, nt, out, ns);
}

__global__ void axpby_kernel(const float* x, const float* z, float* y, float a, float b, int64_t n) {
  for (int64_t i = (int64_t)blockIdx.x * blockDim.x + threadIdx.x; i < n; i += (int64_t)gridDim.x * blockDim.x)
    y[i] = a * x[i] + b * z[i];
}

__device__ __forceinline__ float ln_finish(float v, float mean, float rstd, int c, int b, float mk,
                                           const float* __restrict__ gamma, const float* __restrict__ beta,
                                           const float* __restrict__ shift, const float* __restrict__ scale,
                                           int64_t mod_bs) {
  v = (v - mean) * rstd;
  if (gamma) v = v * gamma[c] + beta[c];
  v *= mk;
  if (scale) v = v * (1.0f + scale[(int64_t)b * mod_bs + c]) + shift[(int64_t)b * mod_bs + c];
  return v;
}

__global__ __launch_bounds__(256) void layernorm_mod_kernel(const float* __restrict__ x, float* __restrict__ y, int C,
                                                            int T, float eps, const float* __restrict__ mask,
                                                            const float* __restrict__ shift,
                                                            const float* __restrict__ scale, int64_t mod_bs,
                                                            const float* __restrict__ gamma,
// ... 276 lines not shown
```

megatts2_hierspeechpp_amd/hierspeechpp_speechsynthesizer.py:

```python
from __future__ import annotations

import math
import os
from typing import Optional

import torch
from torch import nn

from . import _lib as L
from . import commons
from . import functional as Fh
from . import hip_layers
from . import activations
from . import modules
from .alias_free_torch import Activation1d
from .commons import get_padding
from .hip_layers import Conv1d, ConvTranspose1d, Linear, StackedLinearCT, entry as _entry, finalize as _finalize
from .styleencoder import StyleEncoder

UNUSED_PREFIXES = ("enc_p.", "enc_q.", "mel_decoder.", "emb.")

FUSE_ACT_MAX_CHANNELS = int(os.environ.get("HSP_FUSE_ACT_MAX_C", "0"))


class ResidualCouplingBlock_Transformer(nn.Module):

    def __init__(self, channels, hidden_channels, kernel_size, dilation_rate, n_layers=3, n_flows=4, gin_channels=0):
        super().__init__()
        self.channels, self.hidden_channels, self.n_flows = channels, hidden_channels, n_flows
        self.cond_block = nn.ModuleList([Linear(gin_channels, 4 * hidden_channels), nn.Identity(),
                                         Linear(4 * hidden_channels, hidden_channels)])
        self.flows = nn.ModuleList()
        for _ in range(n_flows):
            self.flows.append(modules.ResidualCouplingLayer_Transformer_simple(
                channels, hidden_channels, kernel_size, dilation_rate, n_layers, mean_only=True))
            self.flows.append(modules.Flip())
        lins = [blk.adaLN_modulation[1] for i in range(n_flows) for blk in self.flows[2 * i].enc_block]
        for lin in lins:
            lin.packed = False
        self._mod_rows = lins[0].cout * n_layers
        self.adaln_all = StackedLinearCT(lins)
        if modules.FOLD_FLIP:
            for i in range(n_flows):
                self.flows[2 * i].set_flipped((n_flows - i) % 2 == 1)

    def forward(self, x, x_mask, g=None, reverse=False, owned=False, key_len=None):
        if not reverse:
            raise NotImplementedError("training direction is out of scope")
        c = self.cond_block[0](g.reshape(g.shape[0], -1), act=L.ACT_SILU)
        c_silu = self.cond_block[2](c, act=L.ACT_SILU)
        mods = self.adaln_all(c_silu)
        R = self._mod_rows
        flipped = False
        for i in reversed(range(self.n_flows)):
            layer = self.flows[2 * i]
            if layer.flipped != (not flipped):
                x = self.flows[2 * i + 1](x, x_mask, reverse=True)
                owned = True
            else:
                flipped = not flipped
            x = layer(x, x_mask, g=None, mods=mods[:, i * R:(i + 1) * R], reverse=True, inplace=owned,
                      key_len=key_len)
            owned = True
        return Fh.flip_channels(x) if flipped else x


class PosteriorSFEncoder(nn.Module):

    def __init__(self, src_channels, out_channels, hidden_channels, kernel_size, dilation_rate, n_layers,
                 gin_channels=0):
        super().__init__()
        self.out_channels, self.hidden_channels = out_channels, hidden_channels
        self.pre_source = Conv1d(src_channels, hidden_channels, 1)
        self.pre_filter = Conv1d(1, hidden_channels, 9, stride=4, padding=4)
        self.source_enc = modules.WN(hidden_channels, kernel_size, dilation_rate, n_layers // 2, gin_channels=gin_channels)
        self.filter_enc = modules.WN(hidden_channels, kernel_size, dilation_rate, n_layers // 2, gin_channels=gin_channels)
        self.enc = modules.WN(hidden_channels, kernel_size, dilation_rate, n_layers // 2, gin_channels=gin_channels)
        self.proj = Conv1d(hidden_channels, out_channels * 2, 1)

    def stats(self, x_src, x_ftr, x_mask, g=None):
        x_src = self.pre_source(x_src, mask=x_mask, mask_mode=L.MASK_PRE)
        x_ftr = self.pre_filter(x_ftr, mask=x_mask, mask_mode=L.MASK_PRE)
        x_src = self.source_enc(x_src, x_mask, g=g)
        x_ftr = self.filter_enc(x_ftr, x_mask, g=g)
        x = self.enc(Fh.axpby(x_src, x_ftr, 1.0, 1.0), x_mask, g=g)
        return self.proj(x, mask=x_mask, mask_mode=L.MASK_PRE)

    def forward(self, x_src, x_ftr, x_mask, g=None, noise=None):
        stats = self.stats(x_src, x_ftr, x_mask, g)
        C = self.out_channels
        if noise is None:
            noise = torch.randn(stats.shape[0], C, stats.shape[2], dtype=torch.float32, device=stats.device)
        z = Fh.sample_prior(stats, noise, x_mask, 1.0)
        return z, stats[:, :C], stats[:, C:]


class AMPBlock1(nn.Module):

    def __init__(self, channels, kernel_size=3, dilation=(1, 3, 5), activation=None):
        super().__init__()
        mk = lambda d: Conv1d(channels, channels, kernel_size, dilation=d, padding=get_padding(kernel_size, d),
                              weight_norm=True)
        self.convs1 = nn.ModuleList([mk(d) for d in dilation])
        self.convs2 = nn.ModuleList([mk(1) for _ in dilation])
        for c in list(self.convs1) + list(self.convs2):
            if fft_eligible(channels, kernel_size, c.dilation):
                c.enable_fft()
        self.num_layers = len(self.convs1) + len(self.convs2)
        self.activations = nn.ModuleList([
            Activation1d(activation=activations.SnakeBeta(channels, alpha_logscale=True)) for _ in range(self.num_layers)])

    def forward(self, x, *, out=None, accumulate=False, post_scale=1.0, before_last=None):
        n = len(self.convs1)
        for i, (c1, c2) in enumerate(zip(self.convs1, self.convs2)):
            last = i == n - 1
            x = amp_pair(c1, c2, self.activations[2 * i], self.activations[2 * i + 1], x,
                         before_last=before_last if last else None, res=x, out=out if last else None,
                         accumulate=accumulate and last, post_scale=post_scale if last else 1.0)
        return x


def amp_pair(c1, c2, a1, a2, x, *, form=None, before_last=None, **kw):
    if c1.cin <= FUSE_ACT_MAX_CHANNELS and form is None:
        xt = c1(x, act1d=a1)
        if before_last is not None:
            torch.cuda.current_stream(x.device).wait_event(before_last)
        return c2(xt, act1d=a2, **kw)
    w1 = fft_wins(c1, x) if form is None else form != "direct"
    w2 = fft_wins(c2, x) if form is None else form != "direct"
    if w1 and w2 and fft_act(x) and ((FFT_PAIR and form is None) or form == "pair") and c1.fft_pair_ok(c2, x):
        return c1.forward_fft_pair(c2, x, act_first=a1, act_second=a2, before_inverse=before_last, **kw)
    if form == "pair":
        raise L.HspError("amp_pair(form='pair'): hsp_dftseg_pair_supported says no for this geometry")
    if w1:
        xt = c1.forward_fft(x, act1d=a1) if fft_act(x) else c1.forward_fft(a1(x))
    else:
        xt = c1(a1(x))
    if before_last is not None and not w2:
        torch.cuda.current_stream(x.device).wait_event(before_last)
    if w2:
        return c2.forward_fft(xt, act1d=a2, before_inverse=before_last, **kw) if fft_act(xt) \
            else c2.forward_fft(a2(xt), before_inverse=before_last, **kw)
    return c2(a2(xt), **kw)


FFT_CONV = os.environ.get("HSP_FFT_CONV", "1") == "1"


def fft_eligible(channels: int, k: int, dilation: int) -> bool:
    del dilation
    return channels >= 64 if k >= 11 else (k >= 7 and channels >= 128)


def fft_min_cols(channels: int, k: int) -> int:
    if FFT_MIN_COLS is not None:
        return FFT_MIN_COLS
    if k >= 11:
        return 0 if channels >= 512 else 8000 if channels >= 256 else 32000 if channels >= 128 else 128000
    return 3200 if channels >= 512 else 8000 if channels >= 256 else 64000


FFT_MIN_COLS = int(os.environ["HSP_FFT_MIN_COLS"]) if os.environ.get("HSP_FFT_MIN_COLS") else None
_WARNED_CAPTURE = False


def fft_wins(conv, x) -> bool:
    if not (FFT_CONV and conv._fft and x.stride(2) == 1):
        return False
    B, _, Lx = x.shape
    if B * Lx < fft_min_cols(conv.cin, conv.k):
        return False
    ok = conv._fft_ok
    sup = ok.get((B, Lx))
    if sup is None:
        if len(ok) >= 1024:
            ok.clear()
        sup = ok[(B, Lx)] = conv.fft_supported(B, Lx)
    if sup and (conv._wf is None or conv._wf_form != conv.fft_form()) and torch.cuda.is_current_stream_capturing():
        global _WARNED_CAPTURE
        if not _WARNED_CAPTURE:
            _WARNED_CAPTURE = True
            import warnings
            warnings.warn("a stream capture met a conv whose frequency-domain matrices were never derived: it takes the "
                          "direct form inside this graph (run one eager call or hip_layers.prepare_fft(model) first)")
        return False
    return sup


FFT_ACT = os.environ.get("HSP_FFT_ACT", "1") == "1"
FFT_PAIR = os.environ.get("HSP_FFT_PAIR", "1") == "1"


def fft_act(x) -> bool:
    return FFT_ACT and hip_layers.fft_act_fusable(x)


AMP_STREAMS = int(os.environ.get("HSP_AMP_STREAMS", "1"))
FRONT_SPLITS = int(os.environ.get("HSP_FRONT_SPLITS", "4"))
SERIAL_STREAMS = os.environ.get("HSP_SERIAL_STREAMS", "0") == "1"
_SIDE_STREAMS = {}


def _side_streams(device, n):
    key = (device.type, device.index)
    pool = _SIDE_STREAMS.setdefault(key, [])
    while len(pool) < n:
        pool.append(torch.cuda.Stream(device=device))
    return pool[:n]


def _amp_stage(resblocks, first, num_kernels, x):
    rows = hip_layers.row_lengths()
    if rows is None:
        return _amp_stage_sum(resblocks, first, num_kernels, x)
    rows.prepare(x.shape[2])
    xs = _amp_stage_sum(resblocks, first, num_kernels, x)
    return Fh.mask_mul(xs, rows.mask(xs.shape[2]))


def _amp_stage_sum(resblocks, first, num_kernels, x):
    if not AMP_STREAMS or SERIAL_STREAMS or num_kernels == 1:
        xs = None
        for j in range(num_kernels):
            last = j == num_kernels - 1
            xs = resblocks[first + j](x, out=xs, accumulate=j > 0, post_scale=(1.0 / num_kernels) if last else 1.0)
        return xs
    main = torch.cuda.current_stream(x.device)
    side = _side_streams(x.device, num_kernels - 1)
    xs = torch.empty_like(x)
    fork = torch.cuda.Event()
    fork.record(main)
    done = [torch.cuda.Event() for _ in range(num_kernels)]
    for j in range(num_kernels):
        st = main if j == 0 else side[j - 1]
        last = j == num_kernels - 1
        with torch.cuda.stream(st):
            if j > 0:
                st.wait_event(fork)
            gate = done[j - 1] if j > 0 else None
            resblocks[first + j](x, out=xs, accumulate=j > 0, post_scale=(1.0 / num_kernels) if last else 1.0,
                                 before_last=gate)
            done[j].record(st)
    for ev in done[1:]:
        main.wait_event(ev)
    return xs


class DBlock(nn.Module):

    def __init__(self, input_size, hidden_size, factor):
        super().__init__()
        self.factor = factor
        self.residual_dense = Conv1d(input_size, hidden_size, 1, weight_norm=True)
        self.conv = nn.ModuleList([
            Conv1d(input_size, hidden_size, 3, dilation=1, padding=1, weight_norm=True),
            Conv1d(hidden_size, hidden_size, 3, dilation=2, padding=2, weight_norm=True),
            Conv1d(hidden_size, hidden_size, 3, dilation=4, padding=4, weight_norm=True)])

    def forward(self, x):
        if x.shape[-1] % self.factor != 0:
            raise L.HspError("DBlock needs a length divisible by its factor (pitch is 4 frames per w2v frame)")
        xs = x[..., ::self.factor]
        res = self.residual_dense(xs)
        rows = hip_layers.row_lengths()
        mk = dict(mask=rows.mask(xs.shape[2]), mask_mode=L.MASK_POST) if rows is not None else {}
        h = self.conv[0](xs, lrelu=modules.LRELU_SLOPE, **mk)
        h = self.conv[1](h, lrelu=modules.LRELU_SLOPE, **mk)
        return self.conv[2](h, lrelu=modules.LRELU_SLOPE, res=res)


class SourceNetwork(nn.Module):

    def __init__(self, upsample_initial_channel=256):
        super().__init__()
        ks, us, uks = [3, 5, 7], [2, 2], [4, 4]
        ds = [[1, 3, 5]] * 3
        self.num_kernels, self.num_upsamples = len(ks), len(us)
        c0 = upsample_initial_channel
        self.conv_pre = Conv1d(192, c0, 7, padding=3, weight_norm=True)
        self.ups = nn.ModuleList([ConvTranspose1d(c0 // 2 ** i, c0 // 2 ** (i + 1), k, u, padding=(k - u) // 2,
                                                  weight_norm=True) for i, (u, k) in enumerate(zip(us, uks))])
        self.resblocks = nn.ModuleList()
        for i in range(len(self.ups)):
            ch = c0 // 2 ** (i + 1)
            for k, d in zip(ks, ds):
                self.resblocks.append(AMPBlock1(ch, k, d, activation="snakebeta"))
# ... 224 lines not shown
```

megatts2_hierspeechpp_amd/hip_layers.py:

```python
from __future__ import annotations

import contextvars
import ctypes as C
import os
from typing import Dict, List, Optional, Tuple

import numpy as np
import torch
from torch import nn

from . import _lib as L
from . import functional as Fh
from .synth import kaiser_sinc_filter12


LAUNCH_HOOK = None
DEBUG_FLAGS = 0
FOLD_COLS = os.environ.get("HSP_FOLD_COLS", "1")


_ZEROS = {}


def _zeros(device) -> torch.Tensor:
# ... 5 lines not shown

_DFT = {}


def _dft_tables(device):
    t = _DFT.get(device)
    if t is None:
        n = 4160
        f = np.zeros(n, dtype=np.float32)
        finv = np.zeros(n, dtype=np.float32)
        L.check(L.lib().hsp_dftseg_tables_f32(f.ctypes.data, finv.ctypes.data), "hsp_dftseg_tables_f32")
        t = _DFT[device] = (torch.from_numpy(f).to(device), torch.from_numpy(finv).to(device))
    return t


_TW = {}


def _wspec_twiddles(device):
    t = _TW.get(device)
    if t is None:
        ang = 2.0 * np.pi * np.arange(128, dtype=np.float64) / 128.0
        t = _TW[device] = torch.from_numpy(np.concatenate([np.cos(ang), np.sin(ang)])).to(device)
    return t


FFT_PRODUCT = os.environ.get("HSP_FFT_PRODUCT", "three")


class RowLengths:

    def __init__(self, frames: torch.Tensor, T: int):
        if frames.dtype != torch.int64 or frames.dim() != 1:
            raise L.HspError(f"row lengths must be int64 [B], got {frames.dtype} {tuple(frames.shape)}")
        self.frames, self.T = frames.contiguous(), int(T)
        self._lens: Dict[int, torch.Tensor] = {}
        self._masks: Dict[int, torch.Tensor] = {}

    def factor(self, L_: int) -> int:
        if L_ % self.T != 0:
            raise L.HspError(f"row_exact: a tensor of {L_} columns is not a whole multiple of the {self.T} frames")
        return L_ // self.T

    def at(self, L_: int) -> torch.Tensor:
        t = self._lens.get(L_)
        if t is None:
            f = self.factor(L_)
            t = self._lens[L_] = self.frames if f == 1 else self.frames * f
        return t

    def mask(self, L_: int) -> torch.Tensor:
        m = self._masks.get(L_)
        if m is None:
            m = self._masks[L_] = Fh.sequence_mask(self.at(L_), L_)
        return m

    def prepare(self, L_: int):
        self.at(L_)
        self.mask(L_)


_ROWS: "contextvars.ContextVar[Optional[RowLengths]]" = contextvars.ContextVar("hsp_row_lengths", default=None)


class row_exact:

    def __init__(self, rows: Optional[RowLengths]):
        self.rows = rows

    def __enter__(self):
        self._token = _ROWS.set(self.rows)
        return self.rows

    def __exit__(self, *exc):
        _ROWS.reset(self._token)
        return False


def row_lengths() -> Optional[RowLengths]:
    return _ROWS.get()


def fft_act_fusable(x) -> bool:
    return (x.stride(2) == 1 and x.shape[2] % 4 == 0 and x.stride(0) % 4 == 0 and x.stride(1) % 4 == 0
            and x.data_ptr() % 16 == 0)


SURVEY_ABI = os.environ.get("HSP_SURVEY_ABI", "0") == "1"


def _bracket(kind: str, call, flops: int, nbytes: int, arg, soft: bool = False, span=None):
    hook = LAUNCH_HOOK
    if call is None:
        rc, (e0, e1) = 0, span
    else:
        rc, e0, e1 = L.timed(hook, kind, call, soft)
    if hook is not None and e0 is not None:
        hook(kind, flops, nbytes, e0, e1, arg)
    return rc, e0, e1


class ConvLaunch:
    __slots__ = ("kind", "fn", "args", "flops", "nbytes", "out", "refs")

    def __init__(self, kind, fn, args, flops, nbytes, out, refs):
        self.kind = kind
        self.fn = fn
        self.args = args
        self.flops = flops
        self.nbytes = nbytes
        self.out = out
        self.refs = refs

    def run(self, soft: bool = False) -> int:
        a, fn = self.args, self.fn
        a.debug = DEBUG_FLAGS
        if SURVEY_ABI:
            fn = L.lib().hsp_convtr1d_f32 if a.rows == L.ROWS_SHUFFLE else L.lib().hsp_conv1d_f32
        return _bracket(self.kind, lambda: fn(C.byref(a), L.stream_ptr()), self.flops, self.nbytes, a, soft=soft)[0]


def launch_group(kind: str, fn, launches, *extra):
    live = [p for p in launches if p is not None]
    for p in live:
        p.args.debug = DEBUG_FLAGS
    ptrs = [C.byref(p.args) if p is not None else None for p in launches]
    _bracket(kind, lambda: fn(*ptrs, *extra, L.stream_ptr()), sum(p.flops for p in live), sum(p.nbytes for p in live),
             launches[0].args)


def _set_fold_cols(a) -> None:
    a.fold_cols = 0
    if FOLD_COLS != "0" and a.B > 1 and a.ncols % 4 == 0:
        a.debug = DEBUG_FLAGS
        plan = (C.c_int32 * 4)()
        gated = a.rows in (L.ROWS_GATE_WN, L.ROWS_GATE_GLU)
        if L.lib().hsp_conv1d_mfma_plan(C.byref(a), C.byref(plan)) == 0 and \
                FOLD_COLS in ("1", "gemm" if plan[2] == -2 else "conv") and \
                fold_cols_wanted(plan, a.B, a.ncols, gated=gated, halo=(a.K - 1) * a.dil, act1d=a.prologue == L.PRO_ACT1D):
            a.fold_cols = 1


def fold_cols_kernel(plan, gated: bool = False, halo: int = 0, act1d: bool = False) -> bool:
    bm, bn, kc = int(plan[0]), int(plan[1]), int(plan[2])
    if kc == -2:
        return True
    return kc > 0 and not act1d and halo + 3 <= 64 and (bm, bn) == ((64, 128) if gated else (64, 64))


def fold_cols_wanted(plan, B: int, ncols: int, gated: bool = False, halo: int = 0, act1d: bool = False) -> bool:
    if B < 2 or ncols % 4 != 0 or ncols % int(plan[1]) == 0 or (int(plan[2]) == -2 and int(plan[0]) != 64):
        return False
    return fold_cols_kernel(plan, gated, halo, act1d)


def _round_up(x: int, m: int) -> int:
    return (x + m - 1) // m * m


def plain_rows(cout: int) -> np.ndarray:
    m = _round_up(cout, 4)
    rows = np.full(m, -1, np.int64)
    rows[:cout] = np.arange(cout)
    return rows


def gated_rows(half: int) -> np.ndarray:
    assert half % 32 == 0, "gated convs need a half-width that is a multiple of 32"
    m = np.arange(2 * half)
    return ((m >> 5) & 1) * half + (m >> 6) * 32 + (m & 31)


def conv_pack_map(cout: int, cin: int, k: int, rows: np.ndarray) -> np.ndarray:
    M = rows.shape[0]
    j = np.arange(k)[:, None, None]
    ci = np.arange(cin)[None, :, None]
    co = rows[None, None, :]
    idx = (co * cin + ci) * k + j
    idx = np.where(co >= 0, idx, -1)
    return np.ascontiguousarray(np.broadcast_to(idx, (k, cin, M))).astype(np.int32).reshape(-1)


def convtr_pack_map(cin: int, cout: int, k: int, up: int) -> Tuple[np.ndarray, int, int]:
    kp = -(-k // up)
    M = _round_up(cout * up, 4)
    m = np.arange(M)
    co, r = m // up, m % up
    jp = np.arange(kp)[:, None, None]
    ci = np.arange(cin)[None, :, None]
    tap = r[None, None, :] + (kp - 1 - jp) * up
    idx = (ci * cout + co[None, None, :]) * k + tap
    ok = (tap < k) & (co[None, None, :] < cout)
    return np.where(ok, idx, -1).astype(np.int32).reshape(-1), kp, M


class WeightArena:

    ALIGN = 64

    def __init__(self):
        self.specs: List[Tuple[object, str, int]] = []
        self.buffer: Optional[torch.Tensor] = None
        self.views: Dict[Tuple[int, str], torch.Tensor] = {}
        self._offsets: List[int] = []
        self.total = 0

    def request(self, owner, name: str, numel: int):
        self._offsets.append(self.total)
        self.specs.append((owner, name, numel))
        self.total += _round_up(numel, self.ALIGN)

    def allocate(self, device):
        self.buffer = torch.zeros(max(self.total, 1), dtype=torch.float32, device=device)
        for (owner, name, numel), off in zip(self.specs, self._offsets):
            self.views[(id(owner), name)] = self.buffer[off:off + numel]

    def view(self, owner, name: str) -> torch.Tensor:
        return self.views[(id(owner), name)]


_EPOCH = 0


def _bump_epoch():
    global _EPOCH
    _EPOCH += 1


class HipLayer(nn.Module):

    _hsp_stale = True

    def hsp_requests(self) -> List[Tuple[str, int]]:
        return []

    def hsp_fill(self, arena: WeightArena, materialize: bool) -> None:
        pass

    def _apply(self, fn, *args, **kw):
        before = [(q.device, q.data_ptr()) for q in self._parameters.values() if q is not None]
        r = super()._apply(fn, *args, **kw)
        after = [(q.device, q.data_ptr()) for q in self._parameters.values() if q is not None]
        if before != after:
            self.__dict__["_hsp_stale"] = True
            _bump_epoch()
        return r

    def _load_from_state_dict(self, *args, **kw):
        r = super()._load_from_state_dict(*args, **kw)
        self.__dict__["_hsp_stale"] = True
        _bump_epoch()
        return r


def ensure_ready(model: nn.Module) -> None:
    if model.__dict__.get("_hsp_epoch") == _EPOCH:
        return
    if any(m._hsp_stale for m in model.modules() if isinstance(m, HipLayer)):
        p = next(model.parameters(), None)
        dev = p.device if p is not None else torch.device("cpu")
        if dev.type != "cuda":
            raise L.HspError(f"{type(model).__name__}: parameters are on {dev}; move the model to a ROCm device "
                             "(.cuda() / .to(device)) -- the product path has no CPU fallback")
        fin = getattr(model, "finalize", None)
        if fin is not None:
            fin(dev)
        else:
            finalize(model, dev)
    model.__dict__["_hsp_epoch"] = _EPOCH


def entry(fn):
    import functools

    @functools.wraps(fn)
    def wrapped(self, *args, **kw):
        ensure_ready(self)
        return fn(self, *args, **kw)
    return wrapped


def _gather(src: torch.Tensor, idx_map: np.ndarray, dst: torch.Tensor):
    assert dst.is_contiguous() and src.is_contiguous(), "hsp_gather_f32 reads and writes flat buffers"
    assert idx_map.dtype == np.int32 and idx_map.size == dst.numel() and idx_map.flags["C_CONTIGUOUS"]
    mp = torch.from_numpy(idx_map).to(src.device)
    L.call("hsp_gather_f32", L.fptr(src), L.ptr(mp), L.fptr(dst), dst.numel())
    torch.cuda.current_stream().synchronize()


def _fold(v: torch.Tensor, g: torch.Tensor) -> torch.Tensor:
    rows = v.shape[0]
    cols = v.numel() // rows
    w = torch.empty(v.shape, dtype=v.dtype, device=v.device)
    vc, gc = v.contiguous(), g.contiguous()
    assert gc.numel() == rows
    L.call("hsp_fold_weight_norm_f32", L.fptr(vc), L.fptr(gc), L.fptr(w), rows, cols)
    return w


def _spectrum(Cc: int, Np: int, device) -> torch.Tensor:
    return torch.empty(64, 2 * Cc, Np, dtype=torch.float32, device=device)


class _ConvBase(HipLayer):
    def __init__(self, weight_shape, rows0: int, bias: bool, weight_norm: bool):
        super().__init__()
# ... 125 lines not shown
                self._b.copy_(self._bias_src().flip(0) if self._flip_out else self._bias_src())

    def _fft_args(self, B, Lx):
        d, k = self.dilation, self.k
        hop = 129 - k
        nseg = -(-(-(-Lx // d)) // hop)
        da = L.DftSegArgs()
        da.B, da.C, da.L, da.k, da.dil, da.pad, da.nseg = B, self.cin, Lx, k, d, self.padding, nseg
        da.Np = _round_up(B * d * nseg, 4)
        da.post_scale = 1.0
        da.prod3 = int(self.fft_form() == "three")
        return da

    @staticmethod
    def _fft_point(da, xf, table):
        da.xf, da.xf_bs, da.dft = L.fptr(xf), xf.stride(0), L.fptr(table)

    def _fft_probe(self, B, Lx, dummy=None):
        da = self._fft_args(B, Lx)
        da.xf_bs = 2 * self.cin * da.Np
        da.xf = da.dft = da.act_alpha_exp = da.act_beta_inv = da.act_filt = dummy
        return da

    def fft_supported(self, B, Lx) -> bool:
        return self._fft and bool(L.lib().hsp_dftseg_supported(C.byref(self._fft_probe(B, Lx))))

    @staticmethod
    def _fft_set_act(da, x_like, act1d):
        if act1d._ea is None:
            raise L.HspError("Activation1d used before finalize()")
        da.act_alpha_exp, da.act_beta_inv, da.act_filt = L.fptr(act1d._ea), L.fptr(act1d._binv), L.fptr(act1d._filt)
        rows = _ROWS.get()
        if rows is not None:
            da.act_len = L.ptr(rows.at(x_like.shape[2]))

    def _fft_forward(self, x, act1d=None):
        B, Cc, Lx = x.shape
        assert Cc == self.cin and x.stride(2) == 1 and self._fft
        da = self._fft_args(B, Lx)
        xf = _spectrum(Cc, da.Np, x.device)
        da.x, da.x_bs, da.x_cs = L.fptr(x), x.stride(0), x.stride(1)
        self._fft_point(da, xf, _dft_tables(x.device)[0])
        if act1d is not None:
            if not fft_act_fusable(x):
                raise L.HspError("forward_fft(act1d=...) needs 16-B addressable rows")
            self._fft_set_act(da, x, act1d)
        _, e0, _ = _bracket("hsp_dftseg_fwd_f32", lambda: L.lib().hsp_dftseg_fwd_f32(C.byref(da), L.stream_ptr()),
                            2 * 2 * 64 * 64 * B * Cc * da.dil * da.nseg, 4 * (B * Cc * Lx + 128 * Cc * da.Np), None)
        return xf, e0

    def _fft_product(self, xf):
        Cc, Np = self.cin, xf.shape[2]
        wf = self.ensure_wf()
        yf = _spectrum(Cc, Np, xf.device)
        if self._wf_form == "three":
            pa = L.Cprod3Args()
            pa.xf, pa.yf, pa.w, pa.zeros = L.fptr(xf), L.fptr(yf), L.fptr(wf), L.fptr(_zeros(xf.device))
            pa.xf_bs, pa.yf_bs, pa.bins, pa.C, pa.Np, pa.debug = xf.stride(0), yf.stride(0), 64, Cc, Np, DEBUG_FLAGS
            _bracket("hsp_cprod3_f32", lambda: L.lib().hsp_cprod3_f32(C.byref(pa), L.stream_ptr()),
                     2 * 64 * 3 * Cc * Cc * Np, 4 * (64 * 2 * 2 * Cc * Np + 64 * 3 * Cc * Cc), None)
            return yf
        a = L.Conv1dArgs()
        _set_in(a, xf)
        a.w, a.K, a.dil, a.pad, a.stride = L.fptr(wf), 1, 1, 0, 1
        a.M, a.w_ld, a.w_bs = 2 * Cc, 2 * Cc, 4 * Cc * Cc
        _set_out(a, yf, 64, 2 * Cc, Np)
        a.ncols, a.rows, a.scale, a.post_scale = Np, L.ROWS_PLAIN, 1.0, 1.0
        ConvLaunch("hsp_conv1d_mfma_f32", L.lib().hsp_conv1d_mfma_f32, a, 2 * 64 * 4 * Cc * Cc * Np,
                   4 * (64 * 2 * 2 * Cc * Np + 64 * 4 * Cc * Cc), yf, (xf, yf, wf)).run()
        return yf

    def _fft_inverse_args(self, yf, B, Lx):
        da = self._fft_args(B, Lx)
        self._fft_point(da, yf, _dft_tables(yf.device)[1])
        da.bias = L.fptr(self._b) if self._b is not None else None
        return da

    def _fft_inverse(self, yf, B, Lx, *, res=None, out=None, accumulate=False, post_scale=1.0, before_inverse=None):
        Cc = self.cin
        if out is None:
            out = torch.empty(B, Cc, Lx, dtype=torch.float32, device=yf.device)
        assert out.shape == (B, Cc, Lx) and out.stride(2) == 1 and (res is None or (res.shape == out.shape and res.stride(2) == 1))
        if before_inverse is not None:
            torch.cuda.current_stream(yf.device).wait_event(before_inverse)
        da = self._fft_inverse_args(yf, B, Lx)
        da.y, da.y_bs, da.y_cs = L.fptr(out), out.stride(0), out.stride(1)
        if res is not None:
            da.res, da.res_bs, da.res_cs = L.fptr(res), res.stride(0), res.stride(1)
        da.accumulate, da.post_scale = int(bool(accumulate)), float(post_scale)
        _, _, e1 = _bracket("hsp_dftseg_inv_f32", lambda: L.lib().hsp_dftseg_inv_f32(C.byref(da), L.stream_ptr()),
                            2 * 2 * 64 * 64 * B * Cc * da.dil * da.nseg,
                            4 * (B * Cc * Lx * (self._fft_nio(res, accumulate) - 1) + 128 * Cc * da.Np), None)
        return out, e1

    @staticmethod
    def _fft_nio(res, accumulate) -> int:
        return 2 + bool(res is not None) + 2 * bool(accumulate)

    def _fft_report(self, x, taps, res, accumulate, e_first, e_last, arg):
        B, Cc, Lx = x.shape
        _bracket("hsp_fftconv", None, 2 * B * Cc * Cc * taps * Lx,
                 4 * B * Cc * Lx * self._fft_nio(res, accumulate) + 4 * taps * Cc * Cc, arg, span=(e_first, e_last))

    def forward_fft(self, x, *, res=None, out=None, accumulate=False, post_scale=1.0, act1d=None, before_inverse=None):
        self._require_ready()
        B, _, Lx = x.shape
        xf, e_first = self._fft_forward(x, act1d)
        yf = self._fft_product(xf)
        out, e_last = self._fft_inverse(yf, B, Lx, res=res, out=out, accumulate=accumulate, post_scale=post_scale,
                                        before_inverse=before_inverse)
        self._fft_report(x, self.k, res, accumulate, e_first, e_last, None)
        return out

    def fft_pair_ok(self, second, x) -> bool:
        if not self._fft or not second._fft or second.cin != self.cin or x.shape[2] % 4:
            return False
        B, _, Lx = x.shape
        dummy = L.fptr(_zeros(x.device))
        ia, fa = self._fft_probe(B, Lx, dummy), second._fft_probe(B, Lx, dummy)
        return bool(L.lib().hsp_dftseg_pair_supported(C.byref(ia), C.byref(fa)))

    def _fft_pair_launch(self, second, yf, B, Lx, act_second, like):
        Cc = self.cin
        ia = self._fft_inverse_args(yf, B, Lx)
        fa = second._fft_args(B, Lx)
        xf2 = _spectrum(Cc, fa.Np, yf.device)
        self._fft_point(fa, xf2, _dft_tables(yf.device)[0])
        self._fft_set_act(fa, like, act_second)
        _bracket("hsp_dftseg_pair_f32", lambda: L.lib().hsp_dftseg_pair_f32(C.byref(ia), C.byref(fa), L.stream_ptr()),
                 2 * 2 * 64 * 64 * B * Cc * (ia.dil * ia.nseg + fa.dil * fa.nseg), 4 * 128 * Cc * (ia.Np + fa.Np), None)
        return xf2

    def forward_fft_pair(self, second, x, *, act_first, act_second, res=None, out=None, accumulate=False, post_scale=1.0,
                         before_inverse=None):
        self._require_ready()
        second._require_ready()
        B, _, Lx = x.shape
        xf, e_first = self._fft_forward(x, act_first)
        yf = self._fft_product(xf)
        xf2 = self._fft_pair_launch(second, yf, B, Lx, act_second, x)
        yf2 = second._fft_product(xf2)
        out, e_last = second._fft_inverse(yf2, B, Lx, res=res, out=out, accumulate=accumulate, post_scale=post_scale,
                                          before_inverse=before_inverse)
        self._fft_report(x, self.k + second.k, res, accumulate, e_first, e_last, 2)
        return out

    def prepare(self, x, **kw) -> ConvLaunch:
        if self._pre_norm is not None or "split_out" in kw:
            raise L.HspError("prepare(): split-row and fused-LayerNorm launches go through forward() only")
        return self._prepare(x, **kw)

    def _prepare(self, x, *, act1d=None, lrelu: Optional[float] = None, silu_in=False, act=L.ACT_NONE, cbias=None,
                mask=None, mask_mode=L.MASK_NONE, cscale=None, scale=1.0, res=None, out=None, accumulate=False,
                post_scale=1.0, force_direct=False, row_range=None, split_out=None, mask_mode2=L.MASK_NONE) -> ConvLaunch:
        self._require_ready()
        if act1d is not None and _ROWS.get() is not None:
            raise L.HspError("row_exact: the conv-prologue Activation1d (HSP_FUSE_ACT_MAX_C > 0) has no ragged form")
        B, Cin, Lin = x.shape
        assert Cin == self.cin, (Cin, self.cin)
        gated = self.rows in (L.ROWS_GATE_WN, L.ROWS_GATE_GLU)
        cout = self.cout // 2 if gated else self.cout
        r0 = 0
        if row_range is not None:
            r0, r1 = row_range
            assert not gated and r0 % 4 == 0 and 0 <= r0 < r1 <= self.cout
            cout = r1 - r0
        Lout = (Lin + 2 * self.padding - self.dilation * (self.k - 1) - 1) // self.stride + 1 - self.trim_right
        out2 = None
        if split_out is not None:
            split_row, out2, acc2 = split_out
            assert row_range is None and not gated and self.k == 1 and 0 < split_row < self.cout
            cout = split_row
            if out2 is None:
                assert not acc2
                out2 = torch.empty(B, self.cout - split_row, Lout, dtype=torch.float32, device=x.device)
        if out is None:
            out = torch.empty(B, cout, Lout, dtype=torch.float32, device=x.device)
        a = L.Conv1dArgs()
        _set_in(a, x)
        a.w, a.K, a.dil, a.pad, a.stride = L.fptr(self._w) + 4 * r0, self.k, self.dilation, self.padding, self.stride
        a.M = self.M if row_range is None else _round_up(cout, 4)
        a.w_ld = self.M
        _set_out(a, out, B, cout, Lout)
        a.ncols = Lout
        a.rows, a.gate_half = self.rows, (cout if gated else 0)
        a.bias = (L.fptr(self._b) + 4 * r0) if self._b is not None else None
        _set_epilogue(a, act, cbias, mask, mask_mode, cscale, scale, res, accumulate, post_scale, out)
        if act1d is not None:
            a.prologue = L.PRO_ACT1D
            a.alpha_exp, a.beta_inv, a.filt = L.fptr(act1d._ea), L.fptr(act1d._binv), L.fptr(act1d._filt)
        elif lrelu is not None:
            a.prologue, a.slope = L.PRO_LRELU, float(lrelu)
        elif silu_in:
            a.prologue = L.PRO_SILU
        if self._pre_norm is not None:
            a.ln_c1, a.ln_eps = L.fptr(self._c1), float(self._pre_norm.eps)
            assert not force_direct and row_range is None
        direct = _wants_direct(a, force_direct, silu_in)
        if direct and a.res_ts > 1:
            res = Fh.copy_strided(res)
            a.res, a.res_bs, a.res_cs, a.res_ts = L.fptr(res), res.stride(0), res.stride(1), 0
        rows_full = cout * (2 if gated else 1)
        flops = 2 * B * rows_full * Cin * self.k * Lout
        nbytes = 4 * (B * Cin * Lin + B * cout * Lout * (1 + (res is not None) + bool(accumulate))
                      + rows_full * Cin * self.k)
        if split_out is not None:
            direct = False
            a.Cout = self.cout
            a.split_row, a.accumulate2, a.mask_mode2 = split_row, int(bool(acc2)), mask_mode2
            a.y2, a.y2_bs, a.y2_cs = L.fptr(out2), out2.stride(0), out2.stride(1)
            flops = 2 * B * self.cout * Cin * Lout
            nbytes += 4 * B * (self.cout - split_row) * Lout * (1 + bool(acc2))
        kind, fn = ("hsp_conv1d_direct_f32", L.lib().hsp_conv1d_direct_f32) if direct else \
            ("hsp_conv1d_mfma_f32", L.lib().hsp_conv1d_mfma_f32)
        if not direct:
            _set_fold_cols(a)
        return ConvLaunch(kind, fn, a, flops, nbytes, out if out2 is None else (out, out2),
                          (x, out, out2, res, cbias, mask, cscale))

    def forward(self, x, **kw):
        p = self._prepare(x, **kw)
        if kw.get("split_out") is not None:
            return None if p.run(soft=True) else p.out
        if self._pre_norm is None:
            p.run()
        elif p.run(soft=True):
            xn = Fh.layernorm_mod(x, float(self._pre_norm.eps))
            _set_in(p.args, xn)
            p.args.ln_c1 = None
            _set_fold_cols(p.args)
            p.run()
        return p.out


class ConvTranspose1d(_ConvBase):

    def __init__(self, cin, cout, k, stride, padding=0, bias=True, weight_norm=False):
        super().__init__((cin, cout, k), cin, cout if bias else 0, weight_norm)
        self.cin, self.cout, self.k, self.up, self.padding = cin, cout, k, stride, padding
        self.pack_map, self.kp, self.M = convtr_pack_map(cin, cout, k, stride)

    def hsp_requests(self):
        return [("w", self.kp * self.cin * self.M)] + ([("b", self.cout)] if self.bias is not None else [])

    def hsp_fill(self, arena, materialize):
        self._w = arena.view(self, "w")
        self._b = arena.view(self, "b") if self.bias is not None else None
        if materialize:
            _gather(self._folded(), self.pack_map, self._w)
            if self._b is not None:
                self._b.copy_(self.bias.data)

    def prepare(self, x, *, res=None, out=None, lrelu: Optional[float] = None) -> ConvLaunch:
        self._require_ready()
        B, Cin, Lin = x.shape
        assert Cin == self.cin
        Lout = (Lin - 1) * self.up - 2 * self.padding + self.k
        if out is None:
            out = torch.empty(B, self.cout, Lout, dtype=torch.float32, device=x.device)
        a = L.Conv1dArgs()
        _set_in(a, x)
        a.w, a.K, a.M, a.dil, a.pad, a.stride = L.fptr(self._w), self.kp, self.M, 1, self.kp - 1, 1
        a.w_ld = self.M
        _set_out(a, out, B, self.cout, Lout)
        a.ncols = (Lout - 1 + self.padding) // self.up + 1
        a.rows, a.up, a.shuf_pad = L.ROWS_SHUFFLE, self.up, self.padding
        a.bias = L.fptr(self._b)
        _set_epilogue(a, L.ACT_NONE, None, None, L.MASK_NONE, None, 1.0, res, False, 1.0, out)
        if lrelu is not None:
            a.prologue, a.slope = L.PRO_LRELU, float(lrelu)
        flops = 2 * B * Cin * self.cout * self.k * Lin
        nbytes = 4 * (B * Cin * Lin + B * self.cout * Lout * (1 + (res is not None)) + Cin * self.cout * self.k)
        return ConvLaunch("hsp_conv1d_mfma_f32", L.lib().hsp_conv1d_mfma_f32, a, flops, nbytes, out, (x, out, res))

    def forward(self, x, **kw):
        p = self.prepare(x, **kw)
        p.run()
        return p.out


class _SubArena:

    def __init__(self, arena, owner, prefix):
        self.arena, self.owner, self.prefix = arena, owner, prefix

    def view(self, _layer, name):
        return self.arena.view(self.owner, self.prefix + name)


class PolyphaseConv1d(HipLayer):

    def __init__(self, cin, cout, k, stride, bias=True):
        super().__init__()
        self.cin, self.cout, self.k, self.stride = cin, cout, k, stride
        self.weight = nn.Parameter(torch.zeros(cout, cin, k), requires_grad=False)
        self.bias = nn.Parameter(torch.zeros(cout), requires_grad=False) if bias else None
        ph = [Conv1d(cin, cout, len(range(p, k, stride)), bias=(bias and p == 0)) for p in range(min(stride, k))]
        self.__dict__["_phases"] = ph

    def hsp_requests(self):
        return [(f"p{i}.{n}", numel) for i, ph in enumerate(self._phases) for n, numel in ph.hsp_requests()]

    def hsp_fill(self, arena, materialize):
        for i, ph in enumerate(self._phases):
            if materialize:
                ph.weight.data = self.weight.data[:, :, i::self.stride].contiguous()
                if ph.bias is not None:
                    ph.bias.data = self.bias.data
                ph.to(self.weight.device)
            ph.hsp_fill(_SubArena(arena, self, f"p{i}."), materialize)

    def forward(self, x, **kw):
        B, Cin, Lin = x.shape
        Lout = (Lin - self.k) // self.stride + 1
        out = torch.empty(B, self.cout, Lout, dtype=torch.float32, device=x.device)
        for i, ph in enumerate(self._phases):
            xp = x[:, :, i: i + self.stride * (Lout + ph.k - 1): self.stride]
            ph(xp, out=out, accumulate=i > 0, **(kw if i == len(self._phases) - 1 else {}))
        return out


class GroupedPosConv1d(HipLayer):

    TAPS = 64

    def __init__(self, channels, k, groups):
        super().__init__()
        assert k % 2 == 0 and channels % groups == 0 and k % self.TAPS == 0
        self.channels, self.k, self.groups, self.cg = channels, k, groups, channels // groups
        self.weight_g = nn.Parameter(torch.ones(1, 1, k), requires_grad=False)
        self.weight_v = nn.Parameter(torch.zeros(channels, self.cg, k), requires_grad=False)
        self.bias = nn.Parameter(torch.zeros(channels), requires_grad=False)
        subs = []
        for _ in range(groups):
            for j0 in range(0, k, self.TAPS):
                pad = k // 2 - j0
                c = Conv1d(self.cg, self.cg, self.TAPS, padding=pad, bias=(j0 == 0))
                c.trim_right = 2 * pad - (self.TAPS - 1)
                subs.append(c)
        self.__dict__["_subs"] = subs

    def hsp_requests(self):
        return [(f"s{i}.{n}", numel) for i, c in enumerate(self._subs) for n, numel in c.hsp_requests()]

    def hsp_fill(self, arena, materialize):
        w = None
        nb = self.k // self.TAPS
        if materialize:
            vp = self.weight_v.data.permute(2, 0, 1).contiguous().reshape(self.k, -1)
            w = _fold(vp, self.weight_g.data.reshape(self.k)).reshape(self.k, self.channels, self.cg).permute(1, 2, 0)
        for i, c in enumerate(self._subs):
            gi, bi = divmod(i, nb)
            if materialize:
                c.weight.data = w[gi * self.cg:(gi + 1) * self.cg, :, bi * self.TAPS:(bi + 1) * self.TAPS].contiguous()
                if c.bias is not None:
                    c.bias.data = self.bias.data[gi * self.cg:(gi + 1) * self.cg].contiguous()
            c.hsp_fill(_SubArena(arena, self, f"s{i}."), materialize)

    def forward(self, x):
        nb = self.k // self.TAPS
        conv = torch.empty_like(x)
        for i, c in enumerate(self._subs):
            gi, bi = divmod(i, nb)
            sl = slice(gi * self.cg, (gi + 1) * self.cg)
            c(x[:, sl], out=conv[:, sl], accumulate=bi > 0)
        return Fh.axpby(x, Fh.act(conv, L.ACT_GELU_ERF), 1.0, 1.0)


class Linear(Conv1d):

    def __init__(self, cin, cout, bias=True):
# ... 102 lines not shown
```

Baseline: 35.60 million samples/s.

## Fuse Activation1d (snake anti-aliased) into MFMA conv epilogue for small-channel AMP pairs

Adds an HSP_EPI_ACT epilogue to the MFMA conv kernel. After the conv accumulates, it stages output rows in LDS and applies the upsample, snake and downsample Activation1d in place before writing to global memory. Tiles overlap by 16 columns so each tile carries its own halo. The AMP pair path uses this for the first conv when channels are at most 64 and the plan tile fits. This removes a separate act1d kernel launch and one global round trip of the intermediate tensor, at the cost of recomputing halo columns, more LDS per workgroup and possibly lower occupancy.

```diff
diff --git a/include/hsp.h b/include/hsp.h
--- a/include/hsp.h
+++ b/include/hsp.h
@@ -32,7 +32,8 @@
   HSP_ACT_MISH = 4,
   HSP_ACT_SILU = 5,
   HSP_ACT_SOFTPLUS = 6,
-  HSP_ACT_GELU_ERF = 7
+  HSP_ACT_GELU_ERF = 7,
+  HSP_ACT_ACT1D = 8
 };
 
 enum {
diff --git a/megatts2_hierspeechpp_amd/_lib.py b/megatts2_hierspeechpp_amd/_lib.py
--- a/megatts2_hierspeechpp_amd/_lib.py
+++ b/megatts2_hierspeechpp_amd/_lib.py
@@ -11,6 +11,7 @@
 
 PRO_NONE, PRO_LRELU, PRO_ACT1D, PRO_SILU = 0, 1, 2, 3
 ACT_NONE, ACT_TANH, ACT_GELU_TANH, ACT_RELU, ACT_MISH, ACT_SILU, ACT_SOFTPLUS, ACT_GELU_ERF = 0, 1, 2, 3, 4, 5, 6, 7
+ACT_ACT1D = 8
 ROWS_PLAIN, ROWS_GATE_WN, ROWS_GATE_GLU, ROWS_SHUFFLE = 0, 1, 2, 3
 MASK_NONE, MASK_PRE, MASK_POST, MASK_BOTH = 0, 1, 2, 3
 EINVAL = -1
diff --git a/megatts2_hierspeechpp_amd/csrc/hsp_act1d_arith.h b/megatts2_hierspeechpp_amd/csrc/hsp_act1d_arith.h
--- /dev/null
+++ b/megatts2_hierspeechpp_amd/csrc/hsp_act1d_arith.h
@@ -0,0 +1,38 @@
+#pragma once
+#include "hsp_device.h"
+
+typedef float act_f32x2 __attribute__((ext_vector_type(2)));
+
+#define HSP_ACT2_TAPS(filt, hu, hd)                                              \
+  _Pragma("unroll") for (int i = 0; i < 6; ++i) {                                \
+    (hu)[i] = act_f32x2{2.0f * (filt)[10 - 2 * i], 2.0f * (filt)[11 - 2 * i]};   \
+    (hd)[i] = act_f32x2{(filt)[12 + 2 * i], (filt)[13 + 2 * i]};                 \
+  }
+
+#define HSP_ACT2_UP(a2, raw, pi, hu, kf, kb)                                                                         \
+  {                                                                                                                  \
+    const act_f32x2* rp = reinterpret_cast<const act_f32x2*>((raw) + 2 * (pi) + 2);                                  \
+    const act_f32x2 r0 = rp[0], r1 = rp[1], r2 = rp[2], r3 = rp[3];                                                  \
+    const float xv[7] = {r0.y, r1.x, r1.y, r2.x, r2.y, r3.x, r3.y};                               \
+    act_f32x2 u0 = {0.0f, 0.0f}, u1 = {0.0f, 0.0f};                                                                  \
+    _Pragma("unroll") for (int i = 0; i < 6; ++i) {                                                                  \
+      u0 = __builtin_elementwise_fma(act_f32x2{xv[i], xv[i]}, (hu)[i], u0);                    \
+      u1 = __builtin_elementwise_fma(act_f32x2{xv[i + 1], xv[i + 1]}, (hu)[i], u1);            \
+    }                                                                                                                \
+    *reinterpret_cast<float4*>((a2) + 4 * (pi)) = make_float4(hsp_snake_hw(u0.x, kf, kb), hsp_snake_hw(u0.y, kf, kb), \
+                                                              hsp_snake_hw(u1.x, kf, kb), hsp_snake_hw(u1.y, kf, kb)); \
+  }
+
+#define HSP_ACT2_DOWN(yo, a2, l2, hd)                                                                                \
+  {                                                                                                                  \
+    const float4* ap = reinterpret_cast<const float4*>((a2) + 4 * (l2));                                             \
+    const float4 q0 = ap[0], q1 = ap[1], q2 = ap[2];                                                                 \
+    const act_f32x2 q3 = *reinterpret_cast<const act_f32x2*>((a2) + 4 * (l2) + 12);                                  \
+    const act_f32x2 aw[7] = {{q0.x, q0.y}, {q0.z, q0.w}, {q1.x, q1.y}, {q1.z, q1.w}, {q2.x, q2.y}, {q2.z, q2.w}, q3}; \
+    act_f32x2 s0 = {0.0f, 0.0f}, s1 = {0.0f, 0.0f};                                                                  \
+    _Pragma("unroll") for (int k = 0; k < 6; ++k) {                                                                  \
+      s0 = __builtin_elementwise_fma(aw[k], (hd)[k], s0);                                                            \
+      s1 = __builtin_elementwise_fma(aw[k + 1], (hd)[k], s1);                                                        \
+    }                                                                                                                \
+    (yo) = make_float2(s0.x + s0.y, s1.x + s1.y);                                                                    \
+  }
diff --git a/megatts2_hierspeechpp_amd/csrc/hsp_conv1d_consume.h b/megatts2_hierspeechpp_amd/csrc/hsp_conv1d_consume.h
--- a/megatts2_hierspeechpp_amd/csrc/hsp_conv1d_consume.h
+++ b/megatts2_hierspeechpp_amd/csrc/hsp_conv1d_consume.h
@@ -166,6 +166,18 @@
 #pragma unroll
           for (int r = 0; r < 16; ++r) acc[i][n][r] = 0.0f;
     }
+  } else if constexpr (EPI == HSP_EPI_ACT) {
+    static_for<TM>([&](auto ii) __attribute__((always_inline)) {
+      constexpr int i = decltype(ii)::value;
+      static_for<16>([&](auto rr) __attribute__((always_inline)) {
+        constexpr int r = decltype(rr)::value;
+        const float bz = 0.0f + (a.bias ? a.bias[min(mw + i * 32 + HSP_ACC_ROW(r, half), a.Cout - 1)] : 0.0f);
+        static_for<TN>([&](auto nn) __attribute__((always_inline)) {
+          constexpr int n = decltype(nn)::value;
+          acc[i][n][r] = bz;
+        });
+      });
+    });
   } else {
 #pragma unroll
     for (int i = 0; i < TM; ++i)
@@ -290,7 +302,7 @@
       acc[i][n][r] += red[((i * TN + n) * 16 + r) * 64];
     });
   }
-  if (HSP_DBG(a, HSP_CV_NO_EPILOGUE)) return;
+  if (HSP_DBG(a, HSP_CV_NO_EPILOGUE) && EPI != HSP_EPI_ACT) return;
   if constexpr (EPI == HSP_EPI_INIT) {
     const int mw = L.mw, half = L.half, tw = L.tw, bl = L.bl;
     float* const yb = a.y + (int64_t)bl * a.y_bs;
@@ -333,6 +345,7 @@
   else if constexpr (EPI == HSP_EPI_VEC) epi_vec<FOLD>(a, L, lds, acc);
   else if constexpr (EPI == HSP_EPI_GATE) epi_gate(a, L, acc);
   else if constexpr (EPI == HSP_EPI_SHUF) epi_shuf(a, L, acc);
+  else if constexpr (EPI == HSP_EPI_ACT) EpiAct<C>::consumer(a, L, lds, m0, wm * C::kWN + wn, acc);
   else epi_gen(a, L, acc);
 }
 
diff --git a/megatts2_hierspeechpp_amd/csrc/hsp_conv1d_direct.hip b/megatts2_hierspeechpp_amd/csrc/hsp_conv1d_direct.hip
--- a/megatts2_hierspeechpp_amd/csrc/hsp_conv1d_direct.hip
+++ b/megatts2_hierspeechpp_amd/csrc/hsp_conv1d_direct.hip
@@ -209,6 +209,7 @@
   if (a.w_bs) return HSP_EINVAL;
   if (a.ln_c1 || a.split_row) return HSP_EINVAL;
   if (a.fold_cols) return HSP_EINVAL;
+  if (a.act == HSP_ACT_ACT1D) return HSP_EINVAL;
   if (linear_vec_fast(a)) {
     const unsigned gx = (unsigned)((a.Cout + 63) / 64), gy = (unsigned)((a.B + LV_BB - 1) / LV_BB);
     if (gy > 65535) return HSP_EINVAL;
diff --git a/megatts2_hierspeechpp_amd/csrc/hsp_conv1d_epilogue.h b/megatts2_hierspeechpp_amd/csrc/hsp_conv1d_epilogue.h
--- a/megatts2_hierspeechpp_amd/csrc/hsp_conv1d_epilogue.h
+++ b/megatts2_hierspeechpp_amd/csrc/hsp_conv1d_epilogue.h
@@ -268,4 +268,124 @@
   });
 }
 
-}
+template <class C>
+struct EpiAct {
+  static_assert(C::kWM == 1 && C::kKS == 1 && C::BM % 32 == 0 && C::BN % 256 == 0, "whole rows per consumer wave; float4 row images");
+  static constexpr int BN = C::BN, SEG = C::BN - 16;
+  static constexpr int RIF = BN <= 256 ? 2 : 1;
+  static constexpr int RP = BN <= 256 ? 32 : 16;
+  static constexpr int NPASS = C::BM / RP;
+  static constexpr int NW = C::THREADS / 64;
+  static constexpr int A2W = 2 * BN + 16;
+  static constexpr int NV = BN / 256;
+  static constexpr int NC = (SEG / 2 + 63) / 64;
+  static constexpr int LDS_FLOATS = RP * BN + NW * RIF * A2W;
+  static_assert(RP % (NW * RIF) == 0 && LDS_FLOATS * 4 <= 80 * 1024, "every wave has RIF rows per round; two workgroups per CU");
+
+  static __device__ __forceinline__ void rows(const hsp_conv1d_args& a, float* const lds, int b, int m0, int t0, int pass,
+                                              int wave, int lane, const act_f32x2 (&hu)[6], const act_f32x2 (&hd)[6]) {
+    const int L = a.ncols;
+    const int p0 = t0 + 8;
+    const int n_out = min(SEG, L - p0);
+    for (int rl = wave; rl < RP; rl += NW * RIF) {
+      const int co0 = m0 + pass * RP + rl;
+      if (co0 >= a.Cout) break;
+      float* raw[RIF];
+      float* a2[RIF];
+      float kf[RIF], kb[RIF];
+      bool ok[RIF];
+#pragma unroll
+      for (int j = 0; j < RIF; ++j) {
+        const int co = co0 + NW * j;
+        ok[j] = co < a.Cout;
+        raw[j] = lds + (rl + NW * j) * BN;
+        a2[j] = lds + RP * BN + (wave * RIF + j) * A2W;
+        kf[j] = a.alpha_exp[min(co, a.Cout - 1)] * 0.318309886183790672f;
+        kb[j] = 0.5f * a.beta_inv[min(co, a.Cout - 1)];
+      }
+      if (p0 == 0 || p0 - 8 + BN > L) {
+#pragma unroll
+        for (int j = 0; j < RIF; ++j) {
+          const float x0 = raw[j][8];
+          const float xl = raw[j][min(L - 1 - p0 + 8, BN - 1)];
+          float4 t[NV];
+#pragma unroll
+          for (int v = 0; v < NV; ++v) t[v] = *reinterpret_cast<const float4*>(raw[j] + 4 * (lane + 64 * v));
+          asm volatile("" ::: "memory");
+#pragma unroll
+          for (int v = 0; v < NV; ++v) {
+            const int idx = p0 - 8 + 4 * (lane + 64 * v);
+            t[v] = idx < 0 ? make_float4(x0, x0, x0, x0) : t[v];
+            t[v] = idx >= L ? make_float4(xl, xl, xl, xl) : t[v];
+            *reinterpret_cast<float4*>(raw[j] + 4 * (lane + 64 * v)) = t[v];
+          }
+        }
+        asm volatile("" ::: "memory");
+      }
+      const int npairs = (2 * n_out + 13) >> 2;
+#pragma unroll 2
+      for (int pi = lane; pi < npairs; pi += 64) {
+#pragma unroll
+        for (int j = 0; j < RIF; ++j) HSP_ACT2_UP(a2[j], raw[j], pi, hu, kf[j], kb[j])
+      }
+      asm volatile("" ::: "memory");
+      if (p0 == 0 || p0 + n_out == L) {
+#pragma unroll
+        for (int j = 0; j < RIF; ++j) {
+          if (p0 == 0 && lane < 5) a2[j][lane] = a2[j][5];
+          if (p0 + n_out == L && lane >= 8 && lane < 13) a2[j][2 * n_out + lane - 3] = a2[j][2 * n_out + 4];
+        }
+        asm volatile("" ::: "memory");
+      }
+      float* const yrow = a.y + (int64_t)b * a.y_bs + (int64_t)co0 * a.y_cs + p0;
+#pragma unroll
+      for (int it = 0; it < NC; ++it) {
+        const int l2 = lane + 64 * it;
+        if (2 * l2 >= n_out) continue;
+#pragma unroll
+        for (int j = 0; j < RIF; ++j) {
+          float2 yo;
+          HSP_ACT2_DOWN(yo, a2[j], l2, hd)
+          if (ok[j])
+            __builtin_nontemporal_store(act_f32x2{yo.x, yo.y}, reinterpret_cast<act_f32x2*>(yrow + (int64_t)(NW * j) * a.y_cs + 2 * l2));
+        }
+      }
+      asm volatile("" ::: "memory");
+    }
+  }
+
+  static __device__ __forceinline__ void producer(const hsp_conv1d_args& a, float* const lds, int b, int m0, int t0,
+                                                  int wave, int lane) {
+    act_f32x2 hu[6], hd[6];
+    HSP_ACT2_TAPS(a.filt, hu, hd)
+    for (int pass = 0; pass < NPASS; ++pass) {
+      lds_barrier();
+      rows(a, lds, b, m0, t0, pass, wave, lane, hu, hd);
+      if (pass + 1 < NPASS) lds_barrier();
+    }
+  }
+
+  template <int TM, int TN>
+  static __device__ __forceinline__ void consumer(const hsp_conv1d_args& a, const ConsLane& L, float* const lds, int m0,
+                                                  int wave, const f32x16 (&acc)[TM][TN]) {
+    static_assert(TM * 32 == NPASS * RP, "the passes cover the wave's blocks");
+    act_f32x2 hu[6], hd[6];
+    HSP_ACT2_TAPS(a.filt, hu, hd)
+    float* const col = lds + L.wcol + L.l32;
+    static_for<NPASS>([&](auto pp) __attribute__((always_inline)) {
+      constexpr int pass = pp, i = (pass * RP) / 32, row0 = (pass * RP) % 32;
+      static_for<TN>([&](auto nn) __attribute__((always_inline)) {
+        constexpr int n = nn;
+        static_for<RP / 2>([&](auto rr) __attribute__((always_inline)) {
+          constexpr int r = row0 / 2 + rr;
+          col[(HSP_ACC_ROW(r, L.half) - row0) * BN + 32 * n] = acc[i][n][r];
+        });
+      });
+      lds_barrier();
+      rows(a, lds, L.b, m0, L.t0, pass, wave, L.lane, hu, hd);
+      if (pass + 1 < NPASS) lds_barrier();
+    });
+  }
+};
+
+}
diff --git a/megatts2_hierspeechpp_amd/csrc/hsp_conv1d_mfma.hip b/megatts2_hierspeechpp_amd/csrc/hsp_conv1d_mfma.hip
--- a/megatts2_hierspeechpp_amd/csrc/hsp_conv1d_mfma.hip
+++ b/megatts2_hierspeechpp_amd/csrc/hsp_conv1d_mfma.hip
@@ -35,7 +35,21 @@
   return 0;
 }
 
+int dispatch_epi_act(const hsp_conv1d_args& a, hipStream_t s, int32_t* plan_out) {
+  if (!a.alpha_exp || !a.beta_inv || !a.filt) return HSP_EINVAL;
+  if (a.rows != HSP_ROWS_PLAIN || a.M > 64 || a.Cout > a.M || a.prologue != HSP_PRO_NONE) return HSP_EINVAL;
+  if (a.Lin != a.ncols || a.Lout != a.ncols || 2 * a.pad != (a.K - 1) * a.dil || (a.K - 1) * a.dil > 61 || (a.ncols & 3))
+    return HSP_EINVAL;
+  if (!hsp_aligned16(a.y) || (a.y_bs & 3) || (a.y_cs & 3)) return HSP_EINVAL;
+  if (a.cbias || a.mask_mode != HSP_MASK_NONE || a.cscale || a.res || a.accumulate ||
+      a.scale != 1.0f || a.post_scale != 1.0f)
+    return HSP_EINVAL;
+  if (a.fold_cols || a.w_bs || a.ln_c1 || a.split_row) return HSP_EINVAL;
+  return a.M > 32 ? hsp_conv_tile_M64P(a, HSP_EPI_ACT, false, s, plan_out) : hsp_conv_tile_M32P(a, HSP_EPI_ACT, false, s, plan_out);
+}
+
 int dispatch(const hsp_conv1d_args& a, hipStream_t s, int32_t* plan_out) {
+  if (epi_act_set(a)) return dispatch_epi_act(a, s, plan_out);
   const bool gated = a.rows == HSP_ROWS_GATE_WN || a.rows == HSP_ROWS_GATE_GLU;
   const bool act = a.prologue == HSP_PRO_ACT1D;
   const bool short_seq = hsp_tile_count(a, 128, 128) <= 128;
diff --git a/megatts2_hierspeechpp_amd/csrc/hsp_conv1d_mfma_kernel.h b/megatts2_hierspeechpp_amd/csrc/hsp_conv1d_mfma_kernel.h
--- a/megatts2_hierspeechpp_amd/csrc/hsp_conv1d_mfma_kernel.h
+++ b/megatts2_hierspeechpp_amd/csrc/hsp_conv1d_mfma_kernel.h
@@ -2,6 +2,7 @@
 #include <atomic>
 #include <type_traits>
 #include "hsp_device.h"
+#include "hsp_act1d_arith.h"
 
 typedef float f32x16 __attribute__((ext_vector_type(16)));
 
@@ -38,7 +39,8 @@
   HSP_EPI_VEC = 1,
   HSP_EPI_GATE = 2,
   HSP_EPI_SHUF = 3,
-  HSP_EPI_GEN = 4
+  HSP_EPI_GEN = 4,
+  HSP_EPI_ACT = 5
 };
 
 namespace hspconv {
@@ -173,7 +175,9 @@
     nt = ct % n_nt;
     b = ct / n_nt;
   }
-  const int m0 = mt * BM, t0 = nt * BN;
+  int t0c = nt * BN;
+  if constexpr (EPI == HSP_EPI_ACT) t0c = nt * (BN - 16) - 8;
+  const int m0 = mt * BM, t0 = t0c;
   const int p0 = t0 - a.pad;
   const int ts0 = FOLD ? t0 - b * a.ncols : 0;
 
@@ -242,6 +246,7 @@
           }
           HSP_BARRIER(a);
         }
+        if constexpr (EPI == HSP_EPI_ACT) EpiAct<C>::producer(a, lds, b, m0, t0, wave, lane);
         return;
       }
       PR::dma_w(pa, P, Ws0, 0, m0, pw, lane);
@@ -282,6 +287,7 @@
         HSP_BARRIER(a);
       }
     }
+    if constexpr (EPI == HSP_EPI_ACT) EpiAct<C>::producer(a, lds, b, m0, t0, wave, lane);
     return;
   }
 
@@ -340,9 +346,12 @@
   return (int64_t)a.B * T <= 0x3fffffff;
 }
 
+inline bool epi_act_set(const hsp_conv1d_args& a) { return a.act == HSP_ACT_ACT1D; }
+
 template <class C, int EPI, bool ACT>
 int launch_one(const hsp_conv1d_args& a, hipStream_t s, int32_t* plan_out) {
   if (a.fold_cols && !has_fold_path<C, EPI, ACT>()) return HSP_EINVAL;
+  if (epi_act_set(a) != (EPI == HSP_EPI_ACT)) return HSP_EINVAL;
   const int64_t tiles = (int64_t)((a.M + C::BM - 1) / C::BM) * ((a.ncols + C::BN - 1) / C::BN) * a.B;
   const bool deep_k3 = HSP_DBG(a, HSP_CV_DEEP_K3) && a.K <= 3;
   const bool two_per_cu = !deep_k3 && (C::MINW * 256 >= 2 * C::THREADS || ((tiles > 256 || HSP_DBG(a, HSP_CV_HALF_CU_ANY)) && tiles <= 512 && !HSP_DBG(a, HSP_CV_NO_HALF_CU)));
@@ -350,12 +359,14 @@
   if (lkc < 0) lkc = pick_lkc<C>(a, kMaxLdsBytes);
   if (lkc < 0) return HSP_EINVAL;
   int lds_bytes = make_plan<C>(a.K, a.dil, a.prologue, lkc).total * (int)sizeof(float);
+  if constexpr (EPI == HSP_EPI_ACT) lds_bytes = lds_bytes > EpiAct<C>::LDS_FLOATS * (int)sizeof(float) ? lds_bytes : EpiAct<C>::LDS_FLOATS * (int)sizeof(float);
   if (plan_out) {
     plan_out[0] = C::BM; plan_out[1] = C::BN; plan_out[2] = 1 << lkc; plan_out[3] = lds_bytes;
     return 0;
   }
   const int n_mt = (a.M + C::BM - 1) / C::BM;
-  const int n_nt = (a.ncols + C::BN - 1) / C::BN;
+  constexpr int kColStep = EPI == HSP_EPI_ACT ? C::BN - 16 : C::BN;
+  const int n_nt = (a.ncols + kColStep - 1) / kColStep;
   const int64_t n_ct = (int64_t)n_nt * a.B;
   int g = 0;
   if (HSP_DBG(a, HSP_CV_XCD_GROUPS) && n_mt >= 1 && n_mt <= 8 && (8 % n_mt) == 0) {
diff --git a/megatts2_hierspeechpp_amd/csrc/hsp_conv1d_tile.hip b/megatts2_hierspeechpp_amd/csrc/hsp_conv1d_tile.hip
--- a/megatts2_hierspeechpp_amd/csrc/hsp_conv1d_tile.hip
+++ b/megatts2_hierspeechpp_amd/csrc/hsp_conv1d_tile.hip
@@ -13,6 +13,7 @@
 
 template <int EPI, bool ACT>
 constexpr bool supported() {
+  if (EPI == HSP_EPI_ACT) return !ACT && (same<T, M64P> || same<T, M32P>);
   if (same<T, S64G> || same<T, S64GW> || same<T, S64G2>) return EPI == HSP_EPI_GATE && !ACT;
   if (same<T, M64> || same<T, M32>) return ACT && (EPI == HSP_EPI_INIT || EPI == HSP_EPI_GEN);
   if (ACT) return (same<T, M128> || same<T, S64> || same<T, S64W> || same<T, S32>) && (EPI == HSP_EPI_INIT || EPI == HSP_EPI_GEN);
@@ -43,6 +44,7 @@
     case HSP_EPI_GATE: return by_act<HSP_EPI_GATE>(a, act, s, plan_out);
     case HSP_EPI_SHUF: return by_act<HSP_EPI_SHUF>(a, act, s, plan_out);
     case HSP_EPI_GEN: return by_act<HSP_EPI_GEN>(a, act, s, plan_out);
+    case HSP_EPI_ACT: return by_act<HSP_EPI_ACT>(a, act, s, plan_out);
     default: return HSP_EINVAL;
   }
 }
diff --git a/megatts2_hierspeechpp_amd/csrc/hsp_pointwise.hip b/megatts2_hierspeechpp_amd/csrc/hsp_pointwise.hip
--- a/megatts2_hierspeechpp_amd/csrc/hsp_pointwise.hip
+++ b/megatts2_hierspeechpp_amd/csrc/hsp_pointwise.hip
@@ -1,4 +1,5 @@
 #include "hsp_rows.h"
+#include "hsp_act1d_arith.h"
 
 namespace {
 
@@ -7,8 +8,6 @@
 constexpr int ACT_TILE = 1024;
 constexpr int ACT_THREADS = 256;
 constexpr int ACT_HALO = 8;
-
-typedef float act_f32x2 __attribute__((ext_vector_type(2)));
 
 __global__ __launch_bounds__(ACT_THREADS) void act1d_kernel(const float* __restrict__ x, float* __restrict__ y, int C,
                                                             int L, const float* __restrict__ alpha_exp,
@@ -174,11 +173,7 @@
   float* raw = raw_all[wave];
   float* a2 = a2_all[wave];
   act_f32x2 hu[6], hd[6];
-#pragma unroll
-  for (int i = 0; i < 6; ++i) {
-    hu[i] = act_f32x2{2.0f * filt[10 - 2 * i], 2.0f * filt[11 - 2 * i]};
-    hd[i] = act_f32x2{filt[12 + 2 * i], filt[13 + 2 * i]};
-  }
+  HSP_ACT2_TAPS(filt, hu, hd)
 
   Act2Item cur = act2_item(w0, nseg, C, L);
   float4 rv[2];
@@ -237,17 +232,7 @@
     const int npairs = (2 * n_out + 13) >> 2;
 #pragma unroll 2
     for (int pi = lane; pi < npairs; pi += 64) {
-      const act_f32x2* rp = reinterpret_cast<const act_f32x2*>(raw + 2 * pi + 2);
-      const act_f32x2 r0 = rp[0], r1 = rp[1], r2 = rp[2], r3 = rp[3];
-      const float xv[7] = {r0.y, r1.x, r1.y, r2.x, r2.y, r3.x, r3.y};
-      act_f32x2 u0 = {0.0f, 0.0f}, u1 = {0.0f, 0.0f};
-#pragma unroll
-      for (int i = 0; i < 6; ++i) {
-        u0 = __builtin_elementwise_fma(act_f32x2{xv[i], xv[i]}, hu[i], u0);
-        u1 = __builtin_elementwise_fma(act_f32x2{xv[i + 1], xv[i + 1]}, hu[i], u1);
-      }
-      *reinterpret_cast<float4*>(a2 + 4 * pi) = make_float4(hsp_snake_hw(u0.x, kf, kb), hsp_snake_hw(u0.y, kf, kb),
-                                                            hsp_snake_hw(u1.x, kf, kb), hsp_snake_hw(u1.y, kf, kb));
+      HSP_ACT2_UP(a2, raw, pi, hu, kf, kb)
     }
     act2_compiler_fence();
     if constexpr (RAG) {
@@ -268,17 +253,7 @@
     for (int it = 0; it < NC; ++it) {
       const int l2 = lane + 64 * it;
       if (2 * l2 >= n_out) continue;
-      const float4* ap = reinterpret_cast<const float4*>(a2 + 4 * l2);
-      const float4 q0 = ap[0], q1 = ap[1], q2 = ap[2];
-      const act_f32x2 q3 = *reinterpret_cast<const act_f32x2*>(a2 + 4 * l2 + 12);
-      const act_f32x2 aw[7] = {{q0.x, q0.y}, {q0.z, q0.w}, {q1.x, q1.y}, {q1.z, q1.w}, {q2.x, q2.y}, {q2.z, q2.w}, q3};
-      act_f32x2 s0 = {0.0f, 0.0f}, s1 = {0.0f, 0.0f};
-#pragma unroll
-      for (int k = 0; k < 6; ++k) {
-        s0 = __builtin_elementwise_fma(aw[k], hd[k], s0);
-        s1 = __builtin_elementwise_fma(aw[k + 1], hd[k], s1);
-      }
-      yo[it] = make_float2(s0.x + s0.y, s1.x + s1.y);
+      HSP_ACT2_DOWN(yo[it], a2, l2, hd)
       if constexpr (RAG) {
         yo[it].x = 2 * l2 < n_in ? yo[it].x : 0.0f;
         yo[it].y = 2 * l2 + 1 < n_in ? yo[it].y : 0.0f;
diff --git a/megatts2_hierspeechpp_amd/hierspeechpp_speechsynthesizer.py b/megatts2_hierspeechpp_amd/hierspeechpp_speechsynthesizer.py
--- a/megatts2_hierspeechpp_amd/hierspeechpp_speechsynthesizer.py
+++ b/megatts2_hierspeechpp_amd/hierspeechpp_speechsynthesizer.py
@@ -132,6 +132,14 @@
         return c1.forward_fft_pair(c2, x, act_first=a1, act_second=a2, before_inverse=before_last, **kw)
     if form == "pair":
         raise L.HspError("amp_pair(form='pair'): hsp_dftseg_pair_supported says no for this geometry")
+    if form is None and hip_layers.epi_act_eligible(
+            c1.cin, c1.cout, x.shape[2], fft_first=w1, fft_second=w2,
+            row_exact=hip_layers.row_lengths() is not None,
+            plan=c1.plain_plan(x) if (hip_layers.EPI_ACT and c1.cin == c1.cout <= 64) else None):
+        xt = c1(a1(x), epi_act=a2)
+        if before_last is not None:
+            torch.cuda.current_stream(x.device).wait_event(before_last)
+        return c2(xt, **kw)
     if w1:
         xt = c1.forward_fft(x, act1d=a1) if fft_act(x) else c1.forward_fft(a1(x))
     else:
diff --git a/megatts2_hierspeechpp_amd/hip_layers.py b/megatts2_hierspeechpp_amd/hip_layers.py
--- a/megatts2_hierspeechpp_amd/hip_layers.py
+++ b/megatts2_hierspeechpp_amd/hip_layers.py
@@ -181,6 +181,28 @@
     if B < 2 or ncols % 4 != 0 or ncols % int(plan[1]) == 0 or (int(plan[2]) == -2 and int(plan[0]) != 64):
         return False
     return fold_cols_kernel(plan, gated, halo, act1d)
+
+
+EPI_ACT = os.environ.get("HSP_EPI_ACT", "1") == "1"
+EPI_ACT_TILES = ((32, 512), (64, 256))
+EPI_ACT_FLOPS = 60
+
+
+def epi_act_tiling(ncols: int, bn: int):
+    seg = bn - 16
+    return [(t * seg - 8, t * seg, min(seg, ncols - t * seg)) for t in range(-(-ncols // seg))]
+
+
+def epi_act_plan_ok(plan) -> bool:
+    return int(plan[2]) > 0 and (int(plan[0]), int(plan[1])) in EPI_ACT_TILES
+
+
+def epi_act_eligible(cin: int, cout: int, L_: int, *, fft_first: bool, fft_second: bool, row_exact: bool, plan) -> bool:
+    if not EPI_ACT or fft_first or fft_second or row_exact:
+        return False
+    if cin > 64 or cout > 64 or L_ % 4 != 0:
+        return False
+    return plan is not None and epi_act_plan_ok(plan)
 
 
 def _round_up(x: int, m: int) -> int:
@@ -612,7 +634,8 @@
 
     def _prepare(self, x, *, act1d=None, lrelu: Optional[float] = None, silu_in=False, act=L.ACT_NONE, cbias=None,
                 mask=None, mask_mode=L.MASK_NONE, cscale=None, scale=1.0, res=None, out=None, accumulate=False,
-                post_scale=1.0, force_direct=False, row_range=None, split_out=None, mask_mode2=L.MASK_NONE) -> ConvLaunch:
+                post_scale=1.0, force_direct=False, row_range=None, split_out=None, mask_mode2=L.MASK_NONE,
+                epi_act=None) -> ConvLaunch:
         self._require_ready()
         if act1d is not None and _ROWS.get() is not None:
             raise L.HspError("row_exact: the conv-prologue Activation1d (HSP_FUSE_ACT_MAX_C > 0) has no ragged form")
@@ -671,12 +694,31 @@
             a.y2, a.y2_bs, a.y2_cs = L.fptr(out2), out2.stride(0), out2.stride(1)
             flops = 2 * B * self.cout * Cin * Lout
             nbytes += 4 * B * (self.cout - split_row) * Lout * (1 + bool(acc2))
+        if epi_act is not None:
+            if direct or _ROWS.get() is not None:
+                raise L.HspError("epi_act: the activation epilogue is the MFMA path's, and has no ragged form")
+            if act != L.ACT_NONE or a.prologue != L.PRO_NONE:
+                raise L.HspError("epi_act: no pointwise act and no prologue beside the activation epilogue")
+            a.act = L.ACT_ACT1D
+            a.alpha_exp, a.beta_inv, a.filt = L.fptr(epi_act._ea), L.fptr(epi_act._binv), L.fptr(epi_act._filt)
+            flops += EPI_ACT_FLOPS * B * cout * Lout
         kind, fn = ("hsp_conv1d_direct_f32", L.lib().hsp_conv1d_direct_f32) if direct else \
             ("hsp_conv1d_mfma_f32", L.lib().hsp_conv1d_mfma_f32)
         if not direct:
             _set_fold_cols(a)
         return ConvLaunch(kind, fn, a, flops, nbytes, out if out2 is None else (out, out2),
-                          (x, out, out2, res, cbias, mask, cscale))
+                          (x, out, out2, res, cbias, mask, cscale, epi_act))
+
+    def plain_plan(self, x):
+        key = (tuple(x.shape), x.stride(), x.data_ptr() % 16)
+        cache = self.__dict__.setdefault("_plain_plans", {})
+        if key not in cache:
+            p = self._prepare(x, out=x)
+            plan = (C.c_int32 * 4)()
+            p.args.debug = DEBUG_FLAGS
+            ok = p.kind == "hsp_conv1d_mfma_f32" and L.lib().hsp_conv1d_mfma_plan(C.byref(p.args), C.byref(plan)) == 0
+            cache[key] = tuple(plan) if ok else None
+        return cache[key]
 
     def forward(self, x, **kw):
         p = self._prepare(x, **kw)
```

Result: faster. 36.05 million samples/s, median of 6 (+1.3%).
